# jonathan-laurent/AlphaZero.jl

Hardware: AMD Instinct MI355X
Metric: self-play MCTS sims/sec (Connect-Four, 4096 parallel games per GPU) (higher is better)
Workload: dtype f32

## Files before the change

### alphazero.jl_amd/csrc/net.hip

```cpp
#include "engine.h"

#define AZ_NET_DECL(sfx)                                                                                                     \
  int net_set_kernel_attrs_##sfx(az_engine* e);                                                                                       \
  int net_launch_##sfx(az_engine* e, hipStream_t st, bool from_planes, float* hfeat, const GEnv* envs, const int* eslots,    \
                       const int* n_ptr, int n_max, const float* X, const float* Amask, float* Pout, float* Vout, float* Pinv, \
                       int pstride);                                                                                         \
  int net_wave_##sfx(az_engine* e, int g, bool split, int nmax);                                                             \
  int net_geometry_##sfx(int which, uint16_t* out, int64_t cap, int* rows, int* products);
AZ_NET_DECL(c4)
AZ_NET_DECL(ttt)
AZ_NET_DECL(mancala)
AZ_NET_DECL(go9)

int net_set_kernel_attrs(az_engine* e) {
  switch (e->cfg.game) {
    case AZ_GAME_CONNECT_FOUR: return net_set_kernel_attrs_c4(e);
    case AZ_GAME_TICTACTOE: return net_set_kernel_attrs_ttt(e);
    case AZ_GAME_MANCALA: return net_set_kernel_attrs_mancala(e);
    case AZ_GAME_GO9_PLANES: return net_set_kernel_attrs_go9(e);
  }
  return fail(AZ_ERR_BAD_ARG, "unknown game id %d", e->cfg.game);
}
int net_launch(az_engine* e, hipStream_t st, bool from_planes, float* hfeat, const GEnv* envs, const int* eslots, const int* n_ptr,
               int n_max, const float* X, const float* Amask, float* Pout, float* Vout, float* Pinv, int pstride) {
  switch (e->cfg.game) {
    case AZ_GAME_CONNECT_FOUR: return net_launch_c4(e, st, from_planes, hfeat, envs, eslots, n_ptr, n_max, X, Amask, Pout, Vout, Pinv, pstride);
    case AZ_GAME_TICTACTOE: return net_launch_ttt(e, st, from_planes, hfeat, envs, eslots, n_ptr, n_max, X, Amask, Pout, Vout, Pinv, pstride);
    case AZ_GAME_MANCALA: return net_launch_mancala(e, st, from_planes, hfeat, envs, eslots, n_ptr, n_max, X, Amask, Pout, Vout, Pinv, pstride);
    case AZ_GAME_GO9_PLANES: return net_launch_go9(e, st, from_planes, hfeat, envs, eslots, n_ptr, n_max, X, Amask, Pout, Vout, Pinv, pstride);
  }
  return fail(AZ_ERR_BAD_ARG, "unknown game id %d", e->cfg.game);
}
int net_wave(az_engine* e, int g, bool split, int nmax) {
  switch (e->cfg.game) {
    case AZ_GAME_CONNECT_FOUR: return net_wave_c4(e, g, split, nmax);
    case AZ_GAME_TICTACTOE: return net_wave_ttt(e, g, split, nmax);
    case AZ_GAME_MANCALA: return net_wave_mancala(e, g, split, nmax);
    case AZ_GAME_GO9_PLANES: return net_wave_go9(e, g, split, nmax);
  }
  return fail(AZ_ERR_BAD_ARG, "unknown game id %d", e->cfg.game);
}

extern "C" int az_debug_tower_geometry(int32_t game, int32_t which, uint16_t* out, int64_t cap, int32_t* rows, int32_t* products) {
  if (!out || !rows || !products || which < 0 || which > 3) return fail(AZ_ERR_BAD_ARG, "bad argument");
  switch (game) {
    case AZ_GAME_CONNECT_FOUR: return net_geometry_c4(which, out, cap, rows, products);
    case AZ_GAME_TICTACTOE: return net_geometry_ttt(which, out, cap, rows, products);
    case AZ_GAME_MANCALA: return net_geometry_mancala(which, out, cap, rows, products);
    case AZ_GAME_GO9_PLANES: return net_geometry_go9(which, out, cap, rows, products);
  }
  return fail(AZ_ERR_BAD_ARG, "unknown game id %d", game);
}
```

### alphazero.jl_amd/csrc/net_c4.hip

```cpp
#include "net_impl.h"
AZ_NET_GAME_TU(ConnectFour, c4)


template <int F, int NT> static int tower_timeline(az_engine* e, int32_t n, unsigned long long* out, int64_t cap) {
  using T = T16<ConnectFour, F, NT>;
  const int nb = (n + T::TB - 1) / T::TB;
  if (cap < (int64_t)nb * 8) return fail(AZ_ERR_CAPACITY, "need %d words", nb * 8);
  unsigned long long* d = nullptr;
  AZCHK(dalloc(e, &d, (size_t)nb * 8));
  HIPCHK(hipMemsetAsync(d, 0, sizeof(unsigned long long) * nb * 8, e->stream));
  std::vector<GEnv> envs(n, ConnectFour::init());
  HIPCHK(hipMemcpyAsync(e->d_tmp_env, envs.data(), sizeof(GEnv) * n, hipMemcpyHostToDevice, e->stream));
  HIPCHK(hipMemcpyAsync(e->d_ntmp, &n, sizeof(int), hipMemcpyHostToDevice, e->stream));
  Net16Dev nd = e->net16;
  for (int rep = 0; rep < 2; ++rep) {
    nd.dbg = rep ? d : nullptr;
    hipLaunchKernelGGL((k_tower16<ConnectFour, F, false, NT>), dim3(nb), dim3(T::THREADS), T::BYTES, e->stream, nd, e->d_tmp_env, e->d_iota, e->d_ntmp, n, (const float*)nullptr, e->d_hfeat);
  }
  HIPCHK(hipMemcpyAsync(out, d, sizeof(unsigned long long) * nb * 8, hipMemcpyDeviceToHost, e->stream));
  HIPCHK(hipStreamSynchronize(e->stream));
  e->allocs.pop_back();
  (void)hipFree(d);
  return AZ_OK;
}
static int tower_timeline_split(az_engine* e, int32_t n, unsigned long long* out, int64_t cap) {
  using T = T16S<ConnectFour, 128>;
  const int nb = 2 * ((n + T::TB - 1) / T::TB);
  if (nb > e->num_cu) return fail(AZ_ERR_BAD_ARG, "split tower: at most %d boards", e->num_cu / 2 * T::TB);
  if (cap < (int64_t)nb * 8) return fail(AZ_ERR_CAPACITY, "need %d words", nb * 8);
  unsigned long long* d = nullptr;
  AZCHK(dalloc(e, &d, (size_t)nb * 8));
  std::vector<GEnv> envs(n, ConnectFour::init());
  HIPCHK(hipMemcpyAsync(e->d_tmp_env, envs.data(), sizeof(GEnv) * n, hipMemcpyHostToDevice, e->stream));
  HIPCHK(hipMemcpyAsync(e->d_ntmp, &n, sizeof(int), hipMemcpyHostToDevice, e->stream));
  unsigned long long* xa; unsigned long long ep;
  Net16Dev nd = e->net16;
  for (int rep = 0; rep < 2; ++rep) {
    nd.dbg = rep ? d : nullptr;
    AZCHK(xch_slot<ConnectFour>(e, e->d_hfeat, &xa, &ep));
    hipLaunchKernelGGL((k_tower16s<ConnectFour, 128, false>), dim3(nb), dim3(T::THREADS), T::BYTES, e->stream, nd, e->d_tmp_env, e->d_iota, e->d_ntmp, n, (const float*)nullptr, e->d_hfeat,
                       xa, ep, e->v.err, e->d_xflag);
  }
  HIPCHK(hipMemcpyAsync(out, d, sizeof(unsigned long long) * nb * 8, hipMemcpyDeviceToHost, e->stream));
  HIPCHK(hipStreamSynchronize(e->stream));
  e->allocs.pop_back();
  (void)hipFree(d);
  return AZ_OK;
}
template <int F> static int tower_timeline_bf16(az_engine* e, int32_t n, unsigned long long* out, int64_t cap) {
  using T = T16B<ConnectFour, F, 11>;
  const int nb = (n + T::TB - 1) / T::TB;
  if (cap < (int64_t)nb * 8) return fail(AZ_ERR_CAPACITY, "need %d words", nb * 8);
  unsigned long long* d = nullptr;
  AZCHK(dalloc(e, &d, (size_t)nb * 8));
  std::vector<GEnv> envs(n, ConnectFour::init());
  HIPCHK(hipMemcpyAsync(e->d_tmp_env, envs.data(), sizeof(GEnv) * n, hipMemcpyHostToDevice, e->stream));
  HIPCHK(hipMemcpyAsync(e->d_ntmp, &n, sizeof(int), hipMemcpyHostToDevice, e->stream));
  Net16bDev nd = e->net16b;
  for (int rep = 0; rep < 2; ++rep) {
    nd.dbg = rep ? d : nullptr;
    hipLaunchKernelGGL((k_tower16b<ConnectFour, F, false, 11>), dim3(nb), dim3(T::THREADS), T::BYTES, e->stream, nd, e->d_tmp_env, e->d_iota, e->d_ntmp, n, (const float*)nullptr, e->d_hfeat);
  }
  HIPCHK(hipMemcpyAsync(out, d, sizeof(unsigned long long) * nb * 8, hipMemcpyDeviceToHost, e->stream));
  HIPCHK(hipStreamSynchronize(e->stream));
  e->allocs.pop_back();
  (void)hipFree(d);
  return AZ_OK;
}
template <int F> static int heads_timeline(az_engine* e, int32_t n, unsigned long long* out, int64_t cap) {
  using H = H16<ConnectFour, F, true>;
  const int nb = 2 * ((n + 15) / 16);
  if (cap < (int64_t)nb * H::WAVES * 4) return fail(AZ_ERR_CAPACITY, "need %d words", nb * H::WAVES * 4);
  unsigned long long* d = nullptr;
  AZCHK(dalloc(e, &d, (size_t)nb * H::WAVES * 4));
  std::vector<GEnv> envs(n, ConnectFour::init());
  HIPCHK(hipMemcpyAsync(e->d_tmp_env, envs.data(), sizeof(GEnv) * n, hipMemcpyHostToDevice, e->stream));
  HIPCHK(hipMemcpyAsync(e->d_ntmp, &n, sizeof(int), hipMemcpyHostToDevice, e->stream));
  AZCHK(net_launch(e, e->stream, false, e->d_hfeat, e->d_tmp_env, e->d_iota, e->d_ntmp, n, nullptr, nullptr, e->d_P, e->d_V, nullptr, ConnectFour::A));
  NetDev nd = e->net;
  nd.dbg = d;
  hipLaunchKernelGGL((k_heads16<ConnectFour, F, true>), dim3(nb), dim3(H::THREADS), H::BYTES, e->stream, nd, e->d_tmp_env, e->d_iota, e->d_ntmp, n, (const float*)nullptr, e->d_hfeat, e->d_P, e->d_V, (float*)nullptr, ConnectFour::A);
  HIPCHK(hipMemcpyAsync(out, d, sizeof(unsigned long long) * nb * H::WAVES * 4, hipMemcpyDeviceToHost, e->stream));
  HIPCHK(hipStreamSynchronize(e->stream));
  e->allocs.pop_back();
  (void)hipFree(d);
  return AZ_OK;
}
extern "C" int az_debug_exchange_timeout(az_engine* e) {
  ENGINE(e);
  if (e->cfg.oracle != AZ_ORACLE_RESNET || !e->net_loaded || e->cfg.game != AZ_GAME_CONNECT_FOUR || e->cfg.num_filters != 128 || e->cfg.net_bf16) return fail(AZ_ERR_BAD_ARG, "connect-four, ResNet oracle, 128 filters, fp32");
  using T = T16S<ConnectFour, 128>;
  const int n = 2;
  std::vector<GEnv> envs(n, ConnectFour::init());
  HIPCHK(hipMemcpyAsync(e->d_tmp_env, envs.data(), sizeof(GEnv) * n, hipMemcpyHostToDevice, e->stream));
  HIPCHK(hipMemcpyAsync(e->d_ntmp, &n, sizeof(int), hipMemcpyHostToDevice, e->stream));
  unsigned long long* xa; unsigned long long ep;
  AZCHK(xch_slot<ConnectFour>(e, e->d_hfeat, &xa, &ep));
  hipLaunchKernelGGL((k_tower16s<ConnectFour, 128, false>), dim3(2 * n), dim3(T::THREADS), T::BYTES, e->stream, e->net16, e->d_tmp_env, e->d_iota, e->d_ntmp, n, (const float*)nullptr, e->d_hfeat,
                     xa, ep | (1ull << 63), e->v.err, e->d_xflag);
  return check_device_error(e);
}
extern "C" int az_debug_tree_stamps(az_engine* e, unsigned long long* out) {
  ENGINE(e);
  if (!out) {
    unsigned long long* d = nullptr;
    AZCHK(dalloc(e, &d, 16));
    AZCHK(sync_all(e));
    e->v.dbg = d; e->gv[0].dbg = d;
    return AZ_OK;
  }
  if (!e->gv[0].dbg) return fail(AZ_ERR_STATE, "stamps are not enabled");
  AZCHK(sync_all(e));
  HIPCHK(hipMemcpy(out, e->gv[0].dbg, 16 * sizeof(unsigned long long), hipMemcpyDeviceToHost));
  return AZ_OK;
}
extern "C" int az_debug_heads_timeline(az_engine* e, int32_t n, unsigned long long* out, int64_t cap) {
  ENGINE(e);
  if (e->cfg.oracle != AZ_ORACLE_RESNET || !e->net_loaded || n < 1 || n > e->nn_cap || e->cfg.game != AZ_GAME_CONNECT_FOUR || !e->net.hd16_ok) return fail(AZ_ERR_BAD_ARG, "connect-four, ResNet oracle with 32 head filters");
  return e->cfg.num_filters == 128 ? heads_timeline<128>(e, n, out, cap) : heads_timeline<64>(e, n, out, cap);
}
extern "C" int az_debug_tower_timeline(az_engine* e, int32_t n, int32_t nt, unsigned long long* out, int64_t cap) {
  ENGINE(e);
  if (e->cfg.oracle != AZ_ORACLE_RESNET) return fail(AZ_ERR_BAD_ARG, "the tower timeline needs an engine with the ResNet oracle");
  if (!e->net_loaded || n < 1 || n > e->nn_cap) return fail(AZ_ERR_BAD_ARG, "bad n / no net");
  if (e->cfg.game == AZ_GAME_CONNECT_FOUR && e->cfg.net_bf16 && nt == 11) return e->cfg.num_filters == 128 ? tower_timeline_bf16<128>(e, n, out, cap) : tower_timeline_bf16<64>(e, n, out, cap);
  if (e->cfg.game != AZ_GAME_CONNECT_FOUR || e->cfg.net_bf16 || (nt != 11 && nt != 3 && nt != 2)) return fail(AZ_ERR_BAD_ARG, "connect-four; fp32: nt = 11, 3 or 2 (= split tower), bf16: nt = 11");
  if (nt == 2) return e->cfg.num_filters == 128 ? tower_timeline_split(e, n, out, cap) : fail(AZ_ERR_BAD_ARG, "split tower: 128 filters");
  if (e->cfg.num_filters == 64) return nt == 11 ? tower_timeline<64, 11>(e, n, out, cap) : tower_timeline<64, 3>(e, n, out, cap);
  return nt == 11 ? tower_timeline<128, 11>(e, n, out, cap) : tower_timeline<128, 3>(e, n, out, cap);
}
```

### alphazero.jl_amd/csrc/net_impl.h

```cpp
#pragma once
#include "engine.h"

template <class T> static constexpr double geo_frac() { return T::Geo::tab.cost / (9.0 * (T::RPAD / 16)); }
template <class T_, int ID_, bool OK_, int HIST_> struct FormFp32 {
  using T = T_;
  static constexpr int ID = ID_, HIST = HIST_;
  static constexpr bool OK = OK_, BF16 = false, STOP = false;
  static const Net16Dev& net(const az_engine* e) { return e->net16; }
  static constexpr double frac() { return geo_frac<T>(); }
};
template <class Gm, int F, int NT, int ID_, int HIST_> struct Form16 : FormFp32<T16<Gm, F, NT>, ID_, (NT > 0), HIST_> {
  template <bool FP> static constexpr auto K = &k_tower16<Gm, F, FP, NT>;
  static void name(char* s, size_t n, const char* g) { snprintf(s, n, "k_tower16<%s,%d,NT=%d>", g, F, NT); }
};
template <class Gm, int F> struct FormSplit : FormFp32<T16S<Gm, F>, TW_SPLIT, F == 128, 0> {
  template <bool FP> static constexpr auto K = &k_tower16s<Gm, F, FP>;
  static void name(char* s, size_t n, const char* g) { snprintf(s, n, "k_tower16s<%s,%d>", g, F); }
};
template <class Gm, int F, int NT0, int NT1, int ID_> struct FormPaired : FormFp32<T16P<Gm, F, NT0, NT1>, ID_, F == 64, 2> {
  template <bool FP> static constexpr auto K = &k_tower16x2<Gm, F, FP, NT0, NT1>;
  static constexpr bool STOP = true;
  static void name(char* s, size_t n, const char* g) {
    if (NT0 == 11) snprintf(s, n, "k_tower16x2<%s,%d>", g, F);
    else snprintf(s, n, "k_tower16x2<%s,%d,NT=%d>", g, F, NT0 + NT1);
  }
};
template <class Gm, int F> struct FormPairedC : FormFp32<T16P<Gm, F>, TW_P21C, F == 64, 2> {
  template <bool FP> static constexpr auto K = &k_tower16x2c<Gm, F, FP>;
  static constexpr bool STOP = true;
  static void name(char* s, size_t n, const char* g) { snprintf(s, n, "k_tower16x2c<%s,%d>", g, F); }
};
template <class Gm, int F> struct FormMixed : FormFp32<T16P<Gm, F>, TW_MIXED, F == 64, 2> {
  using T7 = T16P<Gm, F, 10, 9>;
  template <bool FP> static constexpr auto K = &k_tower16x2m<Gm, F, FP>;
  static void name(char* s, size_t n, const char* g) { snprintf(s, n, "k_tower16x2m<%s,%d>", g, F); }
};
template <class Gm, int F> struct Form32 {
  struct T { static constexpr int RPAD = TOWER_ROWS, TB = RPAD / Gm::P, THREADS = TowerCfg<F>::THREADS, BYTES = TowerLds<F>::BYTES; };
  static constexpr int ID = TW_32, HIST = 3;
  static constexpr bool OK = true, BF16 = false, STOP = false;
  template <bool FP> static constexpr auto K = &k_tower<Gm, F, FP>;
  static const NetDev& net(const az_engine* e) { return e->net; }
  static constexpr double frac() { return 1.0; }
  static void name(char* s, size_t n, const char* g) { snprintf(s, n, "k_tower<%s,%d>", g, F); }
};
template <class Gm, int F, int NT, int ID_, int HIST_> struct Form16b {
  using T = T16B<Gm, F, NT>;
  static constexpr int ID = ID_, HIST = HIST_;
  static constexpr bool OK = NT != 22 || F == 128, BF16 = true, STOP = false;
  template <bool FP> static constexpr auto K = &k_tower16b<Gm, F, FP, NT>;
  static const Net16bDev& net(const az_engine* e) { return e->net16b; }
  static constexpr double frac() { return geo_frac<T>(); }
  static void name(char* s, size_t n, const char* g) { snprintf(s, n, "k_tower16b<%s,%d,NT=%d>", g, F, NT); }
};
template <class... D> struct FormList {};
template <class Gm, int F> using Forms = FormList<
    FormSplit<Gm, F>, Form16<Gm, F, NTS<Gm>, TW_NTS, 1>, Form16<Gm, F, NTM<Gm>, TW_NTM, 3>, Form16<Gm, F, 11, TW_11, 2>,
    FormPaired<Gm, F, 11, 10, TW_P21>, FormPaired<Gm, F, 10, 9, TW_P19>, FormPairedC<Gm, F>, Form32<Gm, F>,
    Form16b<Gm, F, NTS<Gm>, TW_NTS, 1>, Form16b<Gm, F, 11, TW_11, 2>, Form16b<Gm, F, 22, TW_B22, 3>>;
template <class D, int F> static constexpr TowerFacts facts() {
  if constexpr (!D::OK) return TowerFacts{D::ID, D::BF16};
  else return TowerFacts{D::ID, D::BF16, true, D::STOP, D::T::TB, D::T::RPAD, D::frac(), D::BF16 && F == 64 ? 2 : 1};
}
template <class Gm, int F, class... D> static TowerTable tower_table(FormList<D...>) {
  static constexpr TowerFacts forms[] = {facts<D, F>()...};
  return TowerTable{forms, (int)sizeof...(D), F, Gm::P, Gm::APAD};
}
template <class Gm, int F> static TowerTable tower_table() { return tower_table<Gm, F>(Forms<Gm, F>{}); }

template <class D, bool FP> static int set_form_attr() {
  if constexpr (D::OK) HIPCHK(hipFuncSetAttribute(reinterpret_cast<const void*>(D::template K<FP>), hipFuncAttributeMaxDynamicSharedMemorySize, D::T::BYTES));
  return AZ_OK;
}
template <class Gm, int F, class... D> static int set_kernel_attrs_f(FormList<D...>) {
  int r = AZ_OK;
  (void)(((r = set_form_attr<D, false>()) == AZ_OK && (r = set_form_attr<D, true>()) == AZ_OK) && ...);
  AZCHK(r);
  AZCHK((set_form_attr<FormMixed<Gm, F>, false>()));
  HIPCHK(hipFuncSetAttribute(reinterpret_cast<const void*>(&k_heads16<Gm, F, true>), hipFuncAttributeMaxDynamicSharedMemorySize, H16<Gm, F, true>::BYTES));
  HIPCHK(hipFuncSetAttribute(reinterpret_cast<const void*>(&k_heads16<Gm, F, false>), hipFuncAttributeMaxDynamicSharedMemorySize, H16<Gm, F, false>::BYTES));
  return AZ_OK;
}
template <class T> static int upload_geo(az_engine* e) {
  using G = typename T::Geo;
  if (e->d_geo[T::GEO]) return AZ_OK;
  std::vector<uint16_t> h((size_t)10 * G::RPAD);
  for (int i = 0; i < G::RPAD; ++i) h[i] = G::tab.pos[i];
  for (int i = 0; i < 9 * G::RPAD; ++i) h[G::RPAD + i] = G::tab.nbr[i];
  uint16_t* d = nullptr;
  AZCHK(dalloc(e, &d, h.size(), false));
  HIPCHK(hipMemcpyAsync(d, h.data(), h.size() * sizeof(uint16_t), hipMemcpyHostToDevice, e->stream));
  HIPCHK(hipStreamSynchronize(e->stream));
  e->d_geo[T::GEO] = d;
  return AZ_OK;
}
template <class D> static int upload_form_geo(az_engine* e) {
  if constexpr (D::OK && D::ID != TW_32) AZCHK((upload_geo<typename D::T>(e)));
  return AZ_OK;
}
template <class... D> static int upload_geos(az_engine* e, FormList<D...>) {
  int r = AZ_OK;
  (void)(((r = upload_form_geo<D>(e)) == AZ_OK) && ...);
  return r;
}
template <class G> static int geometry_out(uint16_t* out, int64_t cap, int* rows, int* products) {
  if (cap < (int64_t)10 * G::RPAD) return fail(AZ_ERR_CAPACITY, "need %d words", 10 * G::RPAD);
  for (int i = 0; i < G::RPAD; ++i) out[i] = G::tab.pos[i];
  for (int i = 0; i < 9 * G::RPAD; ++i) out[G::RPAD + i] = G::tab.nbr[i];
  *rows = G::RPAD; *products = G::tab.cost;
  return AZ_OK;
}
static const char* game_name(const az_engine* e);
static int raise_stop_word(az_engine* e, hipStream_t sn) {
  HIPCHK(hipEventRecord(e->fr_ev[3], sn));
  HIPCHK(hipStreamWaitEvent(e->fr_s[3], e->fr_ev[3], 0));
  hipLaunchKernelGGL(k_set_word, dim3(1), dim3(1), 0, e->fr_s[3], e->d_bg_stop, e->bg_seq);
  return AZ_OK;
}
template <class Gm> static constexpr bool SIMPLE_OK = Gm::A <= 16;
template <class Gm> static int simple_set_kernel_attrs() {
  if constexpr (SIMPLE_OK<Gm>) {
    const int most = (int)sn_lds_bytes(sn_row_words(16 * SN_WAVES * SN_TPW));
    HIPCHK(hipFuncSetAttribute(reinterpret_cast<const void*>(&k_simplenet<Gm, false>), hipFuncAttributeMaxDynamicSharedMemorySize, most));
    HIPCHK(hipFuncSetAttribute(reinterpret_cast<const void*>(&k_simplenet<Gm, true>), hipFuncAttributeMaxDynamicSharedMemorySize, most));
  }
  return AZ_OK;
}
template <class Gm, bool FROM_PLANES>
static int launch_simple(az_engine* e, hipStream_t st, const GEnv* envs, const int* eslots, const int* n_ptr, int n_max, const float* X,
                         const float* Amask, float* Pout, float* Vout, float* Pinv, int pstride) {
  if constexpr (!SIMPLE_OK<Gm>) return fail(AZ_ERR_STATE, "no SimpleNet kernel for this geometry");
  else {
    if (n_max <= 0) return AZ_OK;
    snprintf(e->last_tower, sizeof e->last_tower, "k_simplenet<%s>", game_name(e));
    e->tower_hist[3]++;
    LAUNCH_ON(e, st, AZ_K_TOWER, n_max, (k_simplenet<Gm, FROM_PLANES>), (n_max + SN_ROWS - 1) / SN_ROWS, SN_THREADS, sn_lds_bytes(e->snet.rs), e->snet,
              envs, eslots, n_ptr, n_max, X, Amask, Pout, Vout, Pinv, pstride);
    return AZ_OK;
  }
}
template <class Net> static int wave_frame(az_engine* e, int g, bool split, Net net) {
  hipStream_t st = e->gs[g], sn = e->gt[g];
  if (split) { HIPCHK(hipEventRecord(e->ev_tree[g], st)); HIPCHK(hipStreamWaitEvent(sn, e->ev_tree[g], 0)); }
  AZCHK(net(sn));
  if (split) {
    HIPCHK(hipEventRecord(e->ev_net[g], sn));
    if (!e->ph.fr_on) HIPCHK(hipStreamWaitEvent(st, e->ev_net[g], 0));
  }
  return AZ_OK;
}
struct WaveLeaves { int N; const int* nev; const int* eslots; };
static WaveLeaves wave_leaves(const az_engine* e, int g, int nmax) {
  const DView& v = e->gv[g];
  return WaveLeaves{std::max(1, std::min(v.G, nmax)), v.n_eval + e->wave_par[g], v.eval_slots + (size_t)e->wave_par[g] * v.eval_stride};
}
template <class Gm> static int wave_simple(az_engine* e, int g, bool split, int nmax) {
  const DView& v = e->gv[g];
  const WaveLeaves w = wave_leaves(e, g, nmax);
  return wave_frame(e, g, split, [&](hipStream_t sn) -> int {
    AZCHK((launch_simple<Gm, false>(e, sn, v.leaf_env, w.eslots, w.nev, w.N, nullptr, nullptr, v.Pout, v.Vout, nullptr, Gm::APAD)));
    if (e->bg_signal) AZCHK(raise_stop_word(e, sn));
    return AZ_OK;
  });
}

template <class Gm> static int set_kernel_attrs(az_engine* e) {
  if (e->cfg.oracle == AZ_ORACLE_SIMPLENET) return simple_set_kernel_attrs<Gm>();
  AZCHK((set_kernel_attrs_f<Gm, 64>(Forms<Gm, 64>{})));
  AZCHK((set_kernel_attrs_f<Gm, 128>(Forms<Gm, 128>{})));
  memset(e->d_geo, 0, sizeof e->d_geo);
  AZCHK(upload_geos(e, Forms<Gm, 64>{}));
  AZCHK(upload_geos(e, Forms<Gm, 128>{}));
  AZCHK((upload_geo<typename FormMixed<Gm, 64>::T7>(e)));
  AZCHK((upload_geo<T16<Gm, 64, 6>>(e)));
  return AZ_OK;
}

static TowerAsk tower_ask(const az_engine* e, int n) {
  TowerAsk a;
  a.n = n; a.num_cu = e->num_cu; a.ngroups = e->ngroups;
  a.bf16 = e->cfg.net_bf16 != 0; a.num_blocks = e->cfg.num_blocks; a.tower_pick = e->env.tower_pick; a.use_graphs = e->env.use_graphs != 0; a.split_off = e->split_off;
  a.split_streams = split_streams_on_device(e->device);
  return a;
}
template <class Gm> static int xch_slot(az_engine* e, const float* hfeat, unsigned long long** xch, unsigned long long* epoch) {
  using T = T16S<Gm, 128>;
  const size_t words = (size_t)cus(e->num_cu) * T::XCH_WORDS;
  int slot = AZ_MAX_GROUPS;
  for (int g = 0; g < e->ngroups; ++g) if (hfeat == e->g_hfeat[g]) slot = g;
  if (!e->xch[slot]) {
    AZCHK(dalloc(e, &e->xch[slot], words));
    HIPCHK(hipStreamSynchronize(e->stream));
  }
  if (((e->xch_epoch + 1) & 0xFFFFFFull) == 0) {
    AZCHK(sync_all(e));
    for (int k = 0; k <= AZ_MAX_GROUPS; ++k) if (e->xch[k]) HIPCHK(hipMemset(e->xch[k], 0, words * sizeof(unsigned long long)));
    ++e->xch_epoch;
  }
  *xch = e->xch[slot];
  *epoch = ++e->xch_epoch;
  if (e->env.xch_fail_at > 0 && ++e->xch_launches == e->env.xch_fail_at) *epoch |= 1ull << 63;
  return AZ_OK;
}
template <class Gm, int F>
static int launch_heads(az_engine* e, hipStream_t st, const float* hfeat, const GEnv* envs, const int* eslots, const int* n_ptr, int n_max,
                        const float* Amask, float* Pout, float* Vout, float* Pinv, int pstride) {
  const int tiles = (n_max + 15) / 16;
  switch (choose_heads(e->env.heads_pick, e->net.hd16_ok, e->net.hd_ok, n_max, e->ngroups, e->num_cu)) {
    case HD_16_STAGED:
      LAUNCH_ON(e, st, AZ_K_HEADS, n_max, (k_heads16<Gm, F, true>), 2 * tiles, (H16<Gm, F, true>::THREADS), (H16<Gm, F, true>::BYTES), e->net, envs, eslots, n_ptr, n_max, Amask, hfeat, Pout, Vout, Pinv, pstride);
      break;
    case HD_16:
      LAUNCH_ON(e, st, AZ_K_HEADS, n_max, (k_heads16<Gm, F, false>), tiles, (H16<Gm, F, false>::THREADS), (H16<Gm, F, false>::BYTES), e->net, envs, eslots, n_ptr, n_max, Amask, hfeat, Pout, Vout, Pinv, pstride);
      break;
    case HD_MFMA:
      LAUNCH_ON(e, st, AZ_K_HEADS, n_max, (k_heads_mfma<Gm, F>), (n_max + 31) / 32, 64 * (F / 32 + HEADS_NPT<Gm>), 0, e->net, envs, eslots, n_ptr, n_max, Amask, hfeat, Pout, Vout, Pinv, pstride);
      break;
    case HD_VALU:
      LAUNCH_ON(e, st, AZ_K_HEADS, n_max, (k_heads<Gm, F>), (n_max + 3) / 4, 4 * (F + HEADS_LP<Gm>), 0, e->net, envs, eslots, n_ptr, n_max, Amask, hfeat, Pout, Vout, Pinv, pstride);
      break;
  }
  return AZ_OK;
}
struct TowerIn { float* hfeat; const GEnv* envs; const int* eslots; const int* n_ptr; const float* X; int* xerr; int* stop = nullptr; int stop_val = 0; };
static const char* game_name(const az_engine* e) {
  static const char* const gn[] = {"ConnectFour", "TicTacToe", "Mancala", "Go9Planes"};
  return gn[e->cfg.game];
}
template <class D, bool FROM_PLANES> static int launch_form(az_engine* e, hipStream_t st, int n, const TowerIn& in) {
  if constexpr (!D::OK) return fail(AZ_ERR_STATE, "tower form %d does not exist for this network", (int)D::ID);
  else {
    using T = typename D::T;
    D::name(e->last_tower, sizeof e->last_tower, game_name(e));
    e->tower_hist[D::HIST]++;
    e->next_exec = D::frac();
    const int tiles = (n + T::TB - 1) / T::TB;
    if constexpr (D::ID == TW_SPLIT) {
      unsigned long long* xa; unsigned long long ep;
      AZCHK(xch_slot<typename T::Game>(e, in.hfeat, &xa, &ep));
      LAUNCH_ON(e, st, AZ_K_TOWER, n, (D::template K<FROM_PLANES>), T::SPLIT * tiles, T::THREADS, T::BYTES, D::net(e), in.envs, in.eslots, in.n_ptr, n, in.X, in.hfeat,
                xa, ep, in.xerr, e->d_xflag);
    } else if constexpr (D::STOP)
      LAUNCH_ON(e, st, AZ_K_TOWER, n, (D::template K<FROM_PLANES>), tiles, T::THREADS, T::BYTES, D::net(e), in.envs, in.eslots, in.n_ptr, n, in.X, in.hfeat,
                in.stop, in.stop_val, cus(e->num_cu));
    else
      LAUNCH_ON(e, st, AZ_K_TOWER, n, (D::template K<FROM_PLANES>), tiles, T::THREADS, T::BYTES, D::net(e), in.envs, in.eslots, in.n_ptr, n, in.X, in.hfeat);
    return AZ_OK;
  }
}
template <class Gm, int F, bool FROM_PLANES, class... D>
static int launch_tower(FormList<D...>, az_engine* e, hipStream_t st, int form, int n, const TowerIn& in) {
  const bool bf16 = e->cfg.net_bf16 != 0;
  int r = 1;
  (void)((D::ID == form && D::BF16 == bf16 && ((r = launch_form<D, FROM_PLANES>(e, st, n, in)), true)) || ...);
  return r <= 0 ? r : fail(AZ_ERR_STATE, "no tower form %d", form);
}
template <class Gm, int F, bool FROM_PLANES> static int launch_tower(az_engine* e, hipStream_t st, int form, int n, const TowerIn& in) {
  return launch_tower<Gm, F, FROM_PLANES>(Forms<Gm, F>{}, e, st, form, n, in);
}
template <class Gm, int F, bool FROM_PLANES>
static int launch_net_f(az_engine* e, hipStream_t st, float* hfeat, const GEnv* envs, const int* eslots, const int* n_ptr, int n_max, const float* X,
                        const float* Amask, float* Pout, float* Vout, float* Pinv, int pstride) {
  if (n_max <= 0) return AZ_OK;
  AZCHK((launch_tower<Gm, F, FROM_PLANES>(e, st, choose_tower(tower_table<Gm, F>(), tower_ask(e, n_max)), n_max, TowerIn{hfeat, envs, eslots, n_ptr, X, e->v.err})));
  return launch_heads<Gm, F>(e, st, hfeat, envs, eslots, n_ptr, n_max, Amask, Pout, Vout, Pinv, pstride);
}
template <class Gm, bool FROM_PLANES>
static int launch_net(az_engine* e, hipStream_t st, float* hfeat, const GEnv* envs, const int* eslots, const int* n_ptr, int n_max, const float* X,
                      const float* Amask, float* Pout, float* Vout, float* Pinv, int pstride) {
  if (e->cfg.oracle == AZ_ORACLE_SIMPLENET) return launch_simple<Gm, FROM_PLANES>(e, st, envs, eslots, n_ptr, n_max, X, Amask, Pout, Vout, Pinv, pstride);
  if (e->cfg.num_filters == 128) return launch_net_f<Gm, 128, FROM_PLANES>(e, st, hfeat, envs, eslots, n_ptr, n_max, X, Amask, Pout, Vout, Pinv, pstride);
  return launch_net_f<Gm, 64, FROM_PLANES>(e, st, hfeat, envs, eslots, n_ptr, n_max, X, Amask, Pout, Vout, Pinv, pstride);
}


template <class Gm, int F> static int wave_net_f(az_engine* e, int g, bool split, int nmax) {
  const DView& v = e->gv[g];
  const WaveLeaves w = wave_leaves(e, g, nmax);
  const bool fr = e->ph.fr_on && split;
  auto heads = [&](hipStream_t s) -> int {
    return launch_heads<Gm, F>(e, s, e->g_hfeat[g], v.leaf_env, w.eslots, w.nev, w.N, (const float*)nullptr, v.Pout, v.Vout, (float*)nullptr, Gm::APAD);
  };
  AZCHK(wave_frame(e, g, split, [&](hipStream_t sn) -> int {
    TowerAsk ask = tower_ask(e, w.N);
    ask.fr_on = e->ph.fr_on; ask.fr_kbg = e->ph.fr_kbg; ask.tower_mixed = e->env.tower_mixed; ask.bg_signal = e->bg_signal;
    if (v.nleaf_host) ask.seen = ((volatile int*)e->h_nleaf)[g];
    if (v.needy_host) { ask.needy = ((volatile int*)e->h_needy)[g]; ask.needy_on = true; }
    const WaveTower tw = choose_wave_tower(tower_table<Gm, F>(), ask);
    TowerIn in{e->g_hfeat[g], v.leaf_env, w.eslots, w.nev, nullptr, v.xerr};
    if (tw.tower_stops) { in.stop = e->d_bg_stop; in.stop_val = e->bg_seq; }
    if constexpr (FormMixed<Gm, F>::OK) {
      if (tw.mixed) {
        using M = FormMixed<Gm, F>;
        using T8 = typename M::T; using T7 = typename M::T7;
        const int cu = cus(e->num_cu), first = cu * T8::TB;
        M::name(e->last_tower, sizeof e->last_tower, game_name(e));
        e->tower_hist[M::HIST]++;
        e->next_exec = (first * geo_frac<T8>() + (ask.seen - first) * geo_frac<T7>()) / (double)ask.seen;
        LAUNCH_ON(e, sn, AZ_K_TOWER, w.N, (M::template K<false>), cu + (w.N - first + T7::TB - 1) / T7::TB, T8::THREADS, T8::BYTES, M::net(e), in.envs, in.eslots, in.n_ptr, w.N, in.X, in.hfeat, cu, in.stop, in.stop_val);
      }
    }
    if (!tw.mixed) AZCHK((launch_tower<Gm, F, false>(e, sn, tw.form, w.N, in)));
    if (e->bg_signal && !tw.tower_stops) AZCHK(raise_stop_word(e, sn));
    return fr ? heads(sn) : AZ_OK;
  }));
  return fr ? AZ_OK : heads(e->gs[g]);
}
template <class Gm> static int wave_net(az_engine* e, int g, bool split, int nmax) {
  if (e->cfg.oracle == AZ_ORACLE_SIMPLENET) return wave_simple<Gm>(e, g, split, nmax);
  return e->cfg.num_filters == 128 ? wave_net_f<Gm, 128>(e, g, split, nmax) : wave_net_f<Gm, 64>(e, g, split, nmax);
}

#define AZ_NET_GAME_TU(Gm, sfx)                                                                                              \
  int net_set_kernel_attrs_##sfx(az_engine* e) { return set_kernel_attrs<Gm>(e); }                                                      \
  int net_launch_##sfx(az_engine* e, hipStream_t st, bool from_planes, float* hfeat, const GEnv* envs, const int* eslots,    \
                       const int* n_ptr, int n_max, const float* X, const float* Amask, float* Pout, float* Vout, float* Pinv, \
                       int pstride) {                                                                                        \
    return from_planes ? launch_net<Gm, true>(e, st, hfeat, envs, eslots, n_ptr, n_max, X, Amask, Pout, Vout, Pinv, pstride)  \
                       : launch_net<Gm, false>(e, st, hfeat, envs, eslots, n_ptr, n_max, X, Amask, Pout, Vout, Pinv, pstride); \
  }                                                                                                                          \
  int net_wave_##sfx(az_engine* e, int g, bool split, int nmax) { return wave_net<Gm>(e, g, split, nmax); }                  \
  int net_geometry_##sfx(int which, uint16_t* out, int64_t cap, int* rows, int* products) {                                  \
    return which == 0 ? geometry_out<typename T16<Gm, 64, 11>::Geo>(out, cap, rows, products)                                \
         : which == 1 ? geometry_out<typename T16<Gm, 64, NTS<Gm>>::Geo>(out, cap, rows, products)                                 \
         : which == 2 ? geometry_out<typename T16P<Gm, 64>::Geo>(out, cap, rows, products)                                   \
                      : geometry_out<typename T16B<Gm, 128, 22>::Geo>(out, cap, rows, products);                             \
  }
```

### alphazero.jl_amd/csrc/resnet16.h

```cpp
#pragma once
#include <hip/hip_runtime.h>
#include <stdint.h>
#include "../../include/az_numerics.h"
#include "games.h"
#include "resnet.h"


enum GeoSlot {
  GEO_11,
  GEO_NTS,
  GEO_21,
  GEO_6,
  GEO_NTM,
  GEO_19,
  GEO_22,
  GEO_COUNT
};
struct Net16Dev {
  int nblocks;
  const float* stem_w;
  const float* stem_ss;
  const float4* conv_w;
  const float* conv_ss;
  const float4* head_w;
  const float* head_ss;
  const uint16_t* geo[GEO_COUNT];
  unsigned long long* dbg;
};
static constexpr int GEO_NZ = 8;
template <class Gm, int NTILES, int TBOARDS> struct Geo16 {
  static constexpr int P = Gm::P, W = Gm::W, H = Gm::H, RPAD = NTILES * 16, ROWS = TBOARDS * P, NPADR = RPAD - ROWS;
  static_assert(NPADR >= 0, "boards do not fit the tiles");
  struct Tab {
    uint16_t pos[RPAD];
    uint16_t nbr[9 * RPAD];
    uint16_t tapmask[NTILES];
    int cost;
    int la, lb, lg, off;
  };
  static constexpr int lres(int a, int b, int g, int cell) {
    const int bd = cell / P, q = cell % P;
    return (a * (q % W) + b * (q / W) + g * bd) & 7;
  }
  static constexpr int cls(int q) {
    const int x = q % W, y = q / W;
    if (W >= 2 && x == 0) return 1;
    if (W >= 2 && x == W - 1) return 2;
    if (y == 0) return H == 1 ? 0 : 3;
    if (y == H - 1) return 4;
    return 0;
  }
  static constexpr int valid9(int q) {
    int m = 0;
    for (int tap = 0; tap < 9; ++tap) {
      const int x = q % W + (tap % 3 - 1), y = q / W + (tap / 3 - 1);
      if (x >= 0 && x < W && y >= 0 && y < H) m |= 1 << tap;
    }
    return m;
  }
  struct Order { int ord[5]; };
  static constexpr Order order_of(int order_code) {
    Order o{{0, 1, 2, 3, 4}};
    int pool[4] = {1, 2, 3, 4}, n = 4, code = order_code;
    for (int i = 0; i < 4; ++i) {
      const int k = code % n; code /= n;
      o.ord[1 + i] = pool[k];
      for (int j = k; j + 1 < n; ++j) pool[j] = pool[j + 1];
      --n;
    }
    return o;
  }
  static constexpr int cost_of(int order_code, int padpos) {
    const Order o = order_of(order_code);
    int v9[P] = {}, ncls[5] = {};
    for (int q = 0; q < P; ++q) { v9[q] = valid9(q); ncls[cls(q)]++; }
    int cost = 0, r = 0, mask = 0;
    auto put = [&](int m, int count) {
      for (int k = 0; k < count; ++k) {
        mask |= m;
        if (++r % 16 == 0) { for (int t = 0; t < 9; ++t) cost += (mask >> t) & 1; mask = 0; }
      }
    };
    for (int ci = 0; ci < 5; ++ci) {
      for (int b = 0; b < TBOARDS; ++b)
        for (int q = 0; q < P; ++q) if (cls(q) == o.ord[ci]) put(v9[q], 1);
      if (ci == padpos) put(0, NPADR);
    }
    return cost;
  }
  static constexpr int arrange(int order_code, int padpos, int a, int b, int g, bool same_taps, uint16_t (&out)[RPAD]) {
    const Order o = order_of(order_code);
    int v9[P] = {};
    for (int q = 0; q < P; ++q) v9[q] = valid9(q);
    uint16_t cells[RPAD] = {};
    uint8_t res[RPAD] = {};
    int r = 0, off = 0;
    for (int ci = 0; ci < 5; ++ci) {
      int n = 0;
      for (int bd = 0; bd < TBOARDS; ++bd)
        for (int q = 0; q < P; ++q) if (cls(q) == o.ord[ci]) { cells[n] = (uint16_t)(bd * P + q); res[n] = (uint8_t)lres(a, b, g, bd * P + q); ++n; }
      bool used[RPAD] = {};
      for (int i = 0; i < n; ++i) {
        const int want = (r + i) & 7, v = v9[cells[i] % P];
        out[r + i] = 0xfffe;
        for (int j = 0; j < n; ++j)
          if (!used[j] && res[j] == want && (!same_taps || v9[cells[j] % P] == v)) { out[r + i] = cells[j]; used[j] = true; break; }
      }
      for (int i = 0; i < n; ++i) if (out[r + i] == 0xfffe) {
        const int v = v9[cells[i] % P];
        for (int j = 0; j < n; ++j) if (!used[j] && (!same_taps || v9[cells[j] % P] == v)) { out[r + i] = cells[j]; used[j] = true; ++off; break; }
      }
      r += n;
      if (ci == padpos) for (int k = 0; k < NPADR; ++k) out[r++] = 0xffff;
    }
    return off;
  }
  static constexpr int products(const uint16_t (&pos)[RPAD]) {
    int cost = 0;
    for (int t = 0; t < NTILES; ++t) {
      int m = 0;
      for (int i = 0; i < 16; ++i) if (pos[t * 16 + i] != 0xffff) m |= valid9(pos[t * 16 + i] % P);
      for (int tap = 0; tap < 9; ++tap) cost += (m >> tap) & 1;
    }
    return cost;
  }
  static constexpr int mismatch(int order_code, int padpos, int a, int b, int g) {
    const Order o = order_of(order_code);
    int r = 0, off = 0;
    for (int ci = 0; ci < 5; ++ci) {
      int have[8] = {}, n = 0;
      for (int q = 0; q < P; ++q) if (cls(q) == o.ord[ci])
        for (int bd = 0; bd < TBOARDS; ++bd) { have[(a * (q % W) + b * (q / W) + g * bd) & 7]++; ++n; }
      for (int k = 0; k < 8; ++k) {
        const int need = n / 8 + (((k - r) & 7) < n % 8 ? 1 : 0);
        off += have[k] > need ? have[k] - need : 0;
      }
      r += n;
      if (ci == padpos) r += NPADR;
    }
    return off;
  }
  static constexpr Tab build(int order_code, int padpos) {
    Tab t{};
    int ba = 0, bb = 0, bg = 0, boff = RPAD + 1;
    for (int a = 0; a < 8; ++a)
      for (int b = 0; b < 8; ++b)
        for (int g = 0; g < 8; ++g) {
          const int off = mismatch(order_code, padpos, a, b, g);
          if (off < boff) { boff = off; ba = a; bb = b; bg = g; }
        }
    t.la = ba; t.lb = bb; t.lg = bg;
    t.off = arrange(order_code, padpos, ba, bb, bg, false, t.pos);
    if (products(t.pos) > cost_of(order_code, padpos)) t.off = arrange(order_code, padpos, ba, bb, bg, true, t.pos);
    uint16_t row_of[ROWS > 0 ? ROWS : 1] = {};
    for (int i = 0; i < RPAD; ++i) if (t.pos[i] != 0xffff) row_of[t.pos[i]] = (uint16_t)i;
    for (int i = 0; i < NTILES; ++i) t.tapmask[i] = 0;
    for (int i = 0; i < RPAD; ++i) {
      for (int tap = 0; tap < 9; ++tap) {
        const int dx = tap % 3 - 1, dy = tap / 3 - 1;
        int nb = RPAD + ((i + ba * dx + bb * dy + 16) & 7);
        if (t.pos[i] != 0xffff) {
          const int b = t.pos[i] / P, q = t.pos[i] % P, x = q % W + dx, y = q / W + dy;
          if (x >= 0 && x < W && y >= 0 && y < H) { nb = row_of[b * P + y * W + x]; t.tapmask[i / 16] |= (uint16_t)(1u << tap); }
        }
        t.nbr[tap * RPAD + i] = (uint16_t)nb;
      }
    }
    t.cost = 0;
    for (int i = 0; i < NTILES; ++i) for (int tap = 0; tap < 9; ++tap) t.cost += (t.tapmask[i] >> tap) & 1;
    return t;
  }
  static constexpr Tab best() {
    int bo = 0, bp = 4, bc = cost_of(0, 4);
    for (int oc = 0; oc < 24; ++oc)
      for (int pp = 0; pp < 5; ++pp) {
        const int c = cost_of(oc, pp);
        if (c < bc) { bc = c; bo = oc; bp = pp; }
      }
    return build(bo, bp);
  }
  static constexpr Tab tab = best();
};

template <class Gm> constexpr int NTS = Gm::P <= 48 ? 3 : (Gm::P + 15) / 16;
template <class Gm> constexpr int ntm_of() { for (int nt = 4; nt <= 10; ++nt) if ((16 * nt) % Gm::P == 0) return nt; return Gm::P == 42 ? 6 : 0; }
template <class Gm> constexpr int NTM = ntm_of<Gm>();
template <class Gm, int F = 64, int NT = 11> struct T16 {
  static constexpr int NTILE = NT, RPAD = NTILE * 16;
  static constexpr int TB = RPAD / Gm::P;
  static constexpr int ROWS = TB * Gm::P;
  static constexpr int STRIDE = F + 8;
  static constexpr int BUF = (RPAD + GEO_NZ) * STRIDE;
  static constexpr int PLANES = (RPAD + GEO_NZ) * Gm::C;
  static constexpr int TABLE = (10 * RPAD + 1) / 2;
  static constexpr int BYTES = (BUF + PLANES + TABLE) * 4;
  static constexpr int WAVES = F / 16, THREADS = 64 * WAVES;
  static constexpr int CT = F / 16;
  static constexpr int KH = F / 64;
  static constexpr int SQ = F / 16;
  using Game = Gm;
  using Geo = Geo16<Gm, NTILE, TB>;
  static constexpr GeoSlot GEO = NT == 11 ? GEO_11 : NT == NTS<Gm> ? GEO_NTS : NT == NTM<Gm> ? GEO_NTM : GEO_6;
  static_assert(GEO != GEO_6 || NT == 6, "no table slot for this tile count");
  static constexpr int FILT = F;
};
template <class Gm, int F = 64, int NT0_ = 11, int NT1_ = 10> struct T16P {
  static constexpr int NT0 = NT0_, NT1 = NT1_, NTW = NT0 + NT1, RPAD = NTW * 16;
  static constexpr int TB = RPAD / Gm::P;
  static constexpr int ROWS = TB * Gm::P;
  static constexpr int STRIDE = F + 8;
  static constexpr int BUF = (RPAD + GEO_NZ) * STRIDE;
  static constexpr int PLANES = (RPAD + GEO_NZ) * Gm::C;
  static constexpr int TABLE = (10 * RPAD + 1) / 2;
  static constexpr int BYTES = (BUF + PLANES + TABLE) * 4;
  static constexpr int CT = F / 16, WAVES = 2 * CT, THREADS = 64 * WAVES;
  static constexpr int KH = F / 64, SQ = F / 16;
  using Game = Gm;
  using Geo = Geo16<Gm, NTW, TB>;
  static constexpr GeoSlot GEO = NT0 == 11 ? GEO_21 : GEO_19;
  static_assert(NTW == 21 || NTW == 19, "no table slot for this tile count");
  static constexpr int FILT = F;
};

template <int F> __device__ __forceinline__ int posF(int c) {
  const int G = (c >= F / 2 ? 1 : 0) + 2 * (c & 1), w = (c % (F / 2)) >> 1;
  return (w >> 4) * 64 + ((w >> 2) & 3) * 16 + G * 4 + (w & 3);
}

static constexpr int T16_GMAX = 2;

template <class G, int NT, int TILE0, int KH, int NTAP> struct Steps16 {
  static constexpr int MAXS = 9 * KH * ((NT + 1) / 2);
  struct L {
    int n;
    int8_t tap[MAXS], kh[MAXS], t0[MAXS], t1[MAXS];
    int8_t first[MAXS];
    int8_t next_tap[MAXS];
    int8_t ord[MAXS];
    int8_t first_tap;
  };
  static constexpr L make() {
    L l{};
    l.n = 0; l.first_tap = -1;
    int taps[9] = {}, ntaps = 0;
    for (int tap = 0; tap < 9; ++tap) {
      if (NTAP == 1 && tap != 4) continue;
      bool any = false;
      for (int t = 0; t < NT; ++t) any = any || ((G::tab.tapmask[TILE0 + t] >> tap) & 1);
      if (any) taps[ntaps++] = tap;
    }
    for (int ti = 0; ti < ntaps; ++ti) {
      const int tap = taps[ti];
      if (l.first_tap < 0) l.first_tap = (int8_t)tap;
      int act[NT] = {}, na = 0;
      for (int t = 0; t < NT; ++t) if ((G::tab.tapmask[TILE0 + t] >> tap) & 1) act[na++] = t;
      for (int kh = 0; kh < KH; ++kh)
        for (int i = 0; i < na; i += 2) {
          const int k = l.n++;
          l.tap[k] = (int8_t)tap; l.kh[k] = (int8_t)kh; l.t0[k] = (int8_t)act[i]; l.t1[k] = (int8_t)(i + 1 < na ? act[i + 1] : -1);
          l.first[k] = (kh == 0 && i == 0);
          l.next_tap[k] = (int8_t)(ti + 1 < ntaps ? taps[ti + 1] : -1);
          l.ord[k] = (int8_t)ti;
        }
    }
    return l;
  }
  static constexpr L list = make();
};

template <class T>
__device__ __forceinline__ void load_rows16p(const float* __restrict__ buf, int off0, int off1, bool two, int kh, int g, float4 (&a)[T16_GMAX][4]) {
  const float* p0 = buf + off0 + kh * 64 + g * 4;
#pragma unroll
  for (int q = 0; q < 4; ++q) a[0][q] = *(const float4*)(p0 + q * 16);
  if (two) {
    const float* p1 = buf + off1 + kh * 64 + g * 4;
#pragma unroll
    for (int q = 0; q < 4; ++q) a[1][q] = *(const float4*)(p1 + q * 16);
  }
}
template <int T0, int T1, int KHI, int SQ, int NT>
__device__ __forceinline__ void mfma_tiles16(const float4 (&a)[T16_GMAX][4], const float4 (&bfull)[SQ], f32x4v (&acc)[NT]) {
  const float4* b = bfull + KHI * 4;
#pragma unroll
  for (int q = 0; q < 4; ++q) {
    acc[T0] = __builtin_amdgcn_mfma_f32_16x16x4f32(a[0][q].x, b[q].x, acc[T0], 0, 0, 0);
    if constexpr (T1 >= 0) acc[T1] = __builtin_amdgcn_mfma_f32_16x16x4f32(a[1][q].x, b[q].x, acc[T1], 0, 0, 0);
    acc[T0] = __builtin_amdgcn_mfma_f32_16x16x4f32(a[0][q].y, b[q].y, acc[T0], 0, 0, 0);
    if constexpr (T1 >= 0) acc[T1] = __builtin_amdgcn_mfma_f32_16x16x4f32(a[1][q].y, b[q].y, acc[T1], 0, 0, 0);
    acc[T0] = __builtin_amdgcn_mfma_f32_16x16x4f32(a[0][q].z, b[q].z, acc[T0], 0, 0, 0);
    if constexpr (T1 >= 0) acc[T1] = __builtin_amdgcn_mfma_f32_16x16x4f32(a[1][q].z, b[q].z, acc[T1], 0, 0, 0);
    acc[T0] = __builtin_amdgcn_mfma_f32_16x16x4f32(a[0][q].w, b[q].w, acc[T0], 0, 0, 0);
    if constexpr (T1 >= 0) acc[T1] = __builtin_amdgcn_mfma_f32_16x16x4f32(a[1][q].w, b[q].w, acc[T1], 0, 0, 0);
  }
}
template <class T, class SL, int K, int TILE0>
__device__ __forceinline__ void load_idx16p(const uint16_t* __restrict__ nbr, int lrow, int (&idx)[2]) {
  if constexpr (K < SL::list.n) {
    constexpr int tap = SL::list.tap[K], t0 = SL::list.t0[K], t1 = SL::list.t1[K];
    idx[0] = (int)nbr[tap * T::RPAD + (TILE0 + t0) * 16 + lrow] * T::STRIDE;
    if constexpr (t1 >= 0) idx[1] = (int)nbr[tap * T::RPAD + (TILE0 + t1) * 16 + lrow] * T::STRIDE;
  }
}
template <class T, class SL, int NT, int TILE0, int K>
__device__ __forceinline__ void conv16p_steps(const float* __restrict__ buf, const uint16_t* __restrict__ nbr, const float4* __restrict__ wl,
                                              f32x4v (&acc)[NT], int lrow, int g, float4 (&b0)[T::FILT / 16], float4 (&b1)[T::FILT / 16],
                                              float4 (&aA)[T16_GMAX][4], float4 (&aB)[T16_GMAX][4], int (&idx)[2]) {
  constexpr int F = T::FILT;
  if constexpr (K < SL::list.n) {
    constexpr int kh = SL::list.kh[K], t0 = SL::list.t0[K], t1 = SL::list.t1[K], ord = SL::list.ord[K];
    float4 (&cur)[T16_GMAX][4] = (K & 1) ? aB : aA;
    float4 (&nxt)[T16_GMAX][4] = (K & 1) ? aA : aB;
    float4 (&bc)[F / 16] = (ord & 1) ? b1 : b0;
    float4 (&bn)[F / 16] = (ord & 1) ? b0 : b1;
    if constexpr (SL::list.first[K] && SL::list.next_tap[K] >= 0) {
      constexpr int ntap = SL::list.next_tap[K];
#pragma unroll
      for (int q = 0; q < T::SQ; ++q) bn[q] = wl[(size_t)(ntap * T::CT * T::SQ + q) * 64];
    }
    if constexpr (K + 1 < SL::list.n) {
      load_rows16p<T>(buf, idx[0], idx[1], SL::list.t1[K + 1] >= 0, SL::list.kh[K + 1], g, nxt);
      load_idx16p<T, SL, K + 2, TILE0>(nbr, lrow, idx);
    }
    mfma_tiles16<t0, t1, kh, F / 16, NT>(cur, bc, acc);
    __builtin_amdgcn_sched_barrier(0);
    conv16p_steps<T, SL, NT, TILE0, K + 1>(buf, nbr, wl, acc, lrow, g, b0, b1, aA, aB, idx);
  }
}
template <class T, class G, int NT, int TILE0, int NTAP>
__device__ __forceinline__ void conv16p(const float* __restrict__ buf, const uint16_t* __restrict__ nbr, const float4* __restrict__ wl,
                                        f32x4v (&acc)[NT], int lrow, int g) {
  constexpr int F = T::FILT;
  using SL = Steps16<G, NT, TILE0, T::KH, NTAP>;
  if constexpr (SL::list.n > 0) {
    float4 b0[F / 16], b1[F / 16], aA[T16_GMAX][4], aB[T16_GMAX][4];
    int idx[2] = {0, 0};
    constexpr int tap0 = NTAP == 1 ? 0 : SL::list.first_tap;
#pragma unroll
    for (int q = 0; q < F / 16; ++q) b0[q] = wl[(size_t)(tap0 * T::CT * T::SQ + q) * 64];
    load_idx16p<T, SL, 0, TILE0>(nbr, lrow, idx);
    load_rows16p<T>(buf, idx[0], idx[1], SL::list.t1[0] >= 0, SL::list.kh[0], g, aA);
    load_idx16p<T, SL, 1, TILE0>(nbr, lrow, idx);
    __builtin_amdgcn_sched_barrier(0);
    conv16p_steps<T, SL, NT, TILE0, 0>(buf, nbr, wl, acc, lrow, g, b0, b1, aA, aB, idx);
  }
}

template <int F> struct T16Threads { static constexpr int V = 64 * (F / 16); };

struct NoXch {
  static constexpr int STEM_HALVES = 1;
  static constexpr bool EARLY_PUBLISH = false;
};
enum { DERR_EXCHANGE = 6 };
static constexpr unsigned long long XCH_WAIT_TICKS = 5000000ull;
struct PairXch {
  static constexpr int STEM_HALVES = 2;
  unsigned long long* mine;
  const unsigned long long* theirs;
  uint32_t tag0;
  int* err;
  int* hflag;
  int pch;
  static constexpr bool EARLY_PUBLISH = true;
  template <class T, int NT>
  __device__ __forceinline__ void publish(int step, const float (&ov)[NT][4], int tid) const {
    const uint32_t tag = tag0 + (uint32_t)step;
    unsigned long long* m = mine + (size_t)(step & 1) * NT * 4 * T::THREADS + tid;
#pragma unroll
    for (int t = 0; t < NT; ++t)
#pragma unroll
      for (int i = 0; i < 4; ++i)
        __hip_atomic_store(m + (t * 4 + i) * T::THREADS, ((unsigned long long)tag << 32) | __float_as_uint(ov[t][i]), __ATOMIC_RELAXED, __HIP_MEMORY_SCOPE_AGENT);
  }
  template <class T, int NT, int R0>
  __device__ __forceinline__ void collect(int step, float* __restrict__ buf, int g, int lrow, int tid) const {
    constexpr int THREADS = T::THREADS, F = T::FILT;
    const uint32_t tag = tag0 + (uint32_t)step;
    const unsigned long long* th = theirs + (size_t)(step & 1) * NT * 4 * THREADS + tid;
    unsigned long long pv[NT][4];
    int spins = 0;
    unsigned long long t_start = 0;
    for (;;) {
      bool ok = true;
#pragma unroll
      for (int t = 0; t < NT; ++t)
#pragma unroll
        for (int i = 0; i < 4; ++i) {
          pv[t][i] = __hip_atomic_load(th + (t * 4 + i) * THREADS, __ATOMIC_RELAXED, __HIP_MEMORY_SCOPE_AGENT);
          ok = ok && (uint32_t)(pv[t][i] >> 32) == tag;
        }
      if (ok) break;
      if ((++spins & 255) == 0) {
        const unsigned long long now = wall_clock64();
        if (!t_start) t_start = now;
        else if (now - t_start > XCH_WAIT_TICKS) {
          atomicCAS(err, 0, (int)DERR_EXCHANGE);
          if (hflag) __hip_atomic_store(hflag, 1, __ATOMIC_RELAXED, __HIP_MEMORY_SCOPE_SYSTEM);
          break;
        }
      }
    }
    const int ppos = posF<F>(pch);
#pragma unroll
    for (int t = 0; t < NT; ++t)
#pragma unroll
      for (int i = 0; i < 4; ++i) buf[(R0 + t * 16 + g * 4 + i) * T::STRIDE + ppos] = __uint_as_float((uint32_t)pv[t][i]);
    __syncthreads();
  }
};

template <class T, bool FROM_PLANES, int NT, int TILE0, class X = NoXch>
__device__ __forceinline__ void tower16_wave(const Net16Dev& net, float* __restrict__ buf, const float* __restrict__ planes,
                                             const uint16_t* __restrict__ nbr, const uint16_t* __restrict__ pos, int cw,
                                             int lane, int n, int board0, float* __restrict__ hfeat, const X& xch = X{},
                                             int* stop = nullptr, int stop_val = 0) {
  using Gm = typename T::Game;
  using G = typename T::Geo;
  constexpr int F = T::FILT, P = Gm::P, C = Gm::C, TB = T::TB, STRIDE = T::STRIDE, R0 = TILE0 * 16;
  const int lrow = lane & 15, g = lane >> 4;
  unsigned long long* dbg = (net.dbg && threadIdx.x == 0) ? net.dbg + (size_t)blockIdx.x * 8 : nullptr;
#define AZ_STAMP16(i) do { if (dbg) dbg[i] = __builtin_readcyclecounter(); } while (0)
  AZ_STAMP16(0);
  const int ch = cw * 16 + lrow;
  const int opos = posF<F>(ch);

  f32x4v acc[NT];
  float ov[NT][4];
  float xres[NT][4];
#pragma unroll
  for (int hh = 0; hh < X::STEM_HALVES; ++hh) {
    constexpr int KK = 9 * C, K2 = (KK + 1) / 2, NS = (2 * K2 + 3) / 4;
    const int cws = X::STEM_HALVES == 1 ? cw : hh * (F / 32) + cw % (F / 32);
    const int chs = cws * 16 + lrow, oposs = posF<F>(chs);
#pragma unroll
    for (int t = 0; t < NT; ++t) acc[t] = f32x4v{0.f, 0.f, 0.f, 0.f};
#pragma unroll
    for (int s = 0; s < NS; ++s) {
      const float bw = net.stem_w[(size_t)(cws * NS + s) * 64 + lane];
      const int p = 4 * s + g;
      const int k = (p & 1) * K2 + (p >> 1);
      const bool kin = k < KK && p < 2 * K2;
      const int tap = kin ? k / C : 4, c = kin ? k % C : 0;
#pragma unroll
      for (int tile = 0; tile < NT; ++tile) {
        const int row = kin ? (int)nbr[tap * T::RPAD + R0 + tile * 16 + lrow] : T::RPAD;
        const float a = planes[row * C + c];
        acc[tile] = __builtin_amdgcn_mfma_f32_16x16x4f32(a, bw, acc[tile], 0, 0, 0);
      }
    }
    const float sc = net.stem_ss[chs], sh = net.stem_ss[F + chs];
#pragma unroll
    for (int tile = 0; tile < NT; ++tile)
#pragma unroll
      for (int i = 0; i < 4; ++i) {
        const float v = az_fmaf(acc[tile][i], sc, sh);
        const float r = v > 0.0f ? v : 0.0f;
        buf[(R0 + tile * 16 + g * 4 + i) * STRIDE + oposs] = r;
        if (cws == cw) xres[tile][i] = r;
      }
  }
  __syncthreads();
  AZ_STAMP16(1);

  const size_t LAYER_W = (size_t)9 * T::CT * T::SQ * 64;
  for (int layer = 0; layer < 2 * net.nblocks; ++layer) {
#pragma unroll
    for (int t = 0; t < NT; ++t) acc[t] = f32x4v{0.f, 0.f, 0.f, 0.f};
    int lrow_l = lrow;
    asm volatile("" : "+v"(lrow_l));
    conv16p<T, G, NT, TILE0, 9>(buf, nbr, net.conv_w + (size_t)layer * LAYER_W + (size_t)cw * T::SQ * 64 + lane, acc, lrow_l, g);
    const float sc = net.conv_ss[(size_t)layer * 2 * F + ch], sh = net.conv_ss[(size_t)layer * 2 * F + F + ch];
    if (layer == 2) AZ_STAMP16(4);
    if constexpr (X::EARLY_PUBLISH) {
#pragma unroll
      for (int tile = 0; tile < NT; ++tile)
#pragma unroll
        for (int i = 0; i < 4; ++i) {
          float v = az_fmaf(acc[tile][i], sc, sh);
          if (layer & 1) v = v + xres[tile][i];
          ov[tile][i] = v > 0.0f ? v : 0.0f;
          if (layer & 1) xres[tile][i] = ov[tile][i];
        }
      xch.template publish<T, NT>(layer, ov, threadIdx.x);
      __builtin_amdgcn_s_setprio(2);
      __syncthreads();
      if (layer == 2) AZ_STAMP16(5);
#pragma unroll
      for (int tile = 0; tile < NT; ++tile)
#pragma unroll
        for (int i = 0; i < 4; ++i) buf[(R0 + tile * 16 + g * 4 + i) * STRIDE + opos] = ov[tile][i];
      xch.template collect<T, NT, R0>(layer, buf, g, lrow, threadIdx.x);
    } else {
    __builtin_amdgcn_s_setprio(2);
    __syncthreads();
    if (layer == 2) AZ_STAMP16(5);
    if (!(layer & 1)) {
#pragma unroll
      for (int tile = 0; tile < NT; ++tile)
#pragma unroll
        for (int i = 0; i < 4; ++i) {
          const int a = (R0 + tile * 16 + g * 4 + i) * STRIDE + opos;
          const float v = az_fmaf(acc[tile][i], sc, sh);
          buf[a] = v > 0.0f ? v : 0.0f;
        }
    } else {
#pragma unroll
      for (int tile = 0; tile < NT; ++tile)
#pragma unroll
        for (int i = 0; i < 4; ++i) {
          const int a = (R0 + tile * 16 + g * 4 + i) * STRIDE + opos;
          float v = az_fmaf(acc[tile][i], sc, sh);
          v = v + xres[tile][i];
          xres[tile][i] = v > 0.0f ? v : 0.0f;
          buf[a] = xres[tile][i];
        }
    }
    __syncthreads();
    }
    __builtin_amdgcn_s_setprio(0);
    if (layer == 1 || layer == 2) AZ_STAMP16(5 + layer);
  }
  AZ_STAMP16(2);
  if (stop && threadIdx.x == 0) __hip_atomic_store(stop, stop_val, __ATOMIC_RELAXED, __HIP_MEMORY_SCOPE_AGENT);
#pragma unroll
  for (int t = 0; t < NT; ++t) acc[t] = f32x4v{0.f, 0.f, 0.f, 0.f};
  conv16p<T, G, NT, TILE0, 1>(buf, nbr, net.head_w + (size_t)cw * T::SQ * 64 + lane, acc, lrow, g);
  {
    const float sc = net.head_ss[ch], sh = net.head_ss[F + ch];
    const int nvalid = ((n - board0) < TB ? (n - board0) : TB) * P;
#pragma unroll
    for (int tile = 0; tile < NT; ++tile)
#pragma unroll
      for (int i = 0; i < 4; ++i) {
        const int ps = pos[R0 + tile * 16 + g * 4 + i];
        const float v = az_fmaf(acc[tile][i], sc, sh);
        if (ps < nvalid) hfeat[((size_t)board0 * P + ps) * F + ch] = v > 0.0f ? v : 0.0f;
      }
  }
  AZ_STAMP16(3);
#undef AZ_STAMP16
}

template <class T, bool FROM_PLANES>
__device__ __forceinline__ void tower16_fill(float* __restrict__ buf, float* __restrict__ planes, uint16_t* __restrict__ nbr,
                                             uint16_t* __restrict__ pos, const uint16_t* __restrict__ geo, const GEnv* __restrict__ leaf_env,
                                             const int* __restrict__ eval_slots, const float* __restrict__ X, int n, int board0, int tid) {
  using Gm = typename T::Game;
  constexpr int P = Gm::P, C = Gm::C;
  for (int i = tid; i < T::PLANES; i += T::THREADS) {
    const int row = i / C, c = i % C;
    float val = 0.0f;
    if (row < T::RPAD) {
      const int ps = geo[row];
      if (ps != 0xffff && board0 + ps / P < n) {
        const int b = ps / P, q = ps % P;
        if (FROM_PLANES) val = X[((size_t)(board0 + b) * C + c) * P + q];
        else val = Gm::plane(leaf_env[eval_slots[board0 + b]], q, c);
      }
    }
    planes[i] = val;
  }
  for (int i = tid; i < GEO_NZ * T::STRIDE; i += T::THREADS) buf[T::RPAD * T::STRIDE + i] = 0.0f;
  for (int i = tid; i < T::RPAD; i += T::THREADS) pos[i] = geo[i];
  for (int i = tid; i < 9 * T::RPAD; i += T::THREADS) nbr[i] = geo[T::RPAD + i];
}

template <class Gm, int F, bool FROM_PLANES, int NT = 11>
__global__ void __launch_bounds__(T16Threads<F>::V, 2)
k_tower16(Net16Dev net, const GEnv* __restrict__ leaf_env, const int* __restrict__ eval_slots,
          const int* __restrict__ n_eval_ptr, int n_fixed, const float* __restrict__ X, float* __restrict__ hfeat) {
  using T = T16<Gm, F, NT>;
  extern __shared__ __attribute__((aligned(16))) float lds[];
  float* buf = lds;
  float* planes = lds + T::BUF;
  uint16_t* nbr = (uint16_t*)(planes + T::PLANES);
  uint16_t* pos = nbr + 9 * T::RPAD;
  const int n = FROM_PLANES ? n_fixed : *n_eval_ptr;
  const int board0 = blockIdx.x * T::TB;
  if (board0 >= n) return;
  tower16_fill<T, FROM_PLANES>(buf, planes, nbr, pos, net.geo[T::GEO], leaf_env, eval_slots, X, n, board0, threadIdx.x);
  __syncthreads();
  tower16_wave<T, FROM_PLANES, NT, 0>(net, buf, planes, nbr, pos, threadIdx.x >> 6, threadIdx.x & 63, n, board0, hfeat);
}

template <class T, bool FROM_PLANES>
__device__ __forceinline__ void tower16x2_body(const Net16Dev& net, const GEnv* __restrict__ leaf_env, const int* __restrict__ eval_slots, int n,
                                               const float* __restrict__ X, float* __restrict__ hfeat, int board0, const uint16_t* __restrict__ geo,
                                               int* stop = nullptr, int stop_val = 0) {
  extern __shared__ __attribute__((aligned(16))) float lds[];
  float* buf = lds;
  float* planes = lds + T::BUF;
  uint16_t* nbr = (uint16_t*)(planes + T::PLANES);
  uint16_t* pos = nbr + 9 * T::RPAD;
  tower16_fill<T, FROM_PLANES>(buf, planes, nbr, pos, geo, leaf_env, eval_slots, X, n, board0, threadIdx.x);
  __syncthreads();
  const int wave = threadIdx.x >> 6, lane = threadIdx.x & 63;
  if (wave < T::CT) tower16_wave<T, FROM_PLANES, T::NT0, 0>(net, buf, planes, nbr, pos, wave, lane, n, board0, hfeat, NoXch{}, stop, stop_val);
  else tower16_wave<T, FROM_PLANES, T::NT1, T::NT0>(net, buf, planes, nbr, pos, wave - T::CT, lane, n, board0, hfeat);
}
__device__ __forceinline__ int* paired_last_round(int* stop, int wg, int nwg, int num_cu) {
  return stop && wg >= (nwg - 1) / num_cu * num_cu ? stop : nullptr;
}
template <class Gm, int F, bool FROM_PLANES, int NT0 = 11, int NT1 = 10>
__global__ void __launch_bounds__(2 * T16Threads<F>::V, 1)
k_tower16x2(Net16Dev net, const GEnv* __restrict__ leaf_env, const int* __restrict__ eval_slots,
            const int* __restrict__ n_eval_ptr, int n_fixed, const float* __restrict__ X, float* __restrict__ hfeat,
            int* stop, int stop_val, int num_cu) {
  using T = T16P<Gm, F, NT0, NT1>;
  const int n = FROM_PLANES ? n_fixed : *n_eval_ptr;
  const int board0 = blockIdx.x * T::TB;
  if (board0 >= n) return;
  tower16x2_body<T, FROM_PLANES>(net, leaf_env, eval_slots, n, X, hfeat, board0, net.geo[T::GEO], paired_last_round(stop, blockIdx.x, (n + T::TB - 1) / T::TB, num_cu), stop_val);
}
template <class Gm, int F, bool FROM_PLANES>
__global__ void __launch_bounds__(2 * T16Threads<F>::V, 1) __attribute__((amdgpu_num_vgpr(88)))
k_tower16x2c(Net16Dev net, const GEnv* __restrict__ leaf_env, const int* __restrict__ eval_slots,
             const int* __restrict__ n_eval_ptr, int n_fixed, const float* __restrict__ X, float* __restrict__ hfeat,
             int* stop, int stop_val, int num_cu) {
  using T = T16P<Gm, F, 11, 10>;
  const int n = FROM_PLANES ? n_fixed : *n_eval_ptr;
  const int board0 = blockIdx.x * T::TB;
  if (board0 >= n) return;
  tower16x2_body<T, FROM_PLANES>(net, leaf_env, eval_slots, n, X, hfeat, board0, net.geo[T::GEO], paired_last_round(stop, blockIdx.x, (n + T::TB - 1) / T::TB, num_cu), stop_val);
}
template <class Gm, int F, bool FROM_PLANES>
__global__ void __launch_bounds__(2 * T16Threads<F>::V, 1)
k_tower16x2m(Net16Dev net, const GEnv* __restrict__ leaf_env, const int* __restrict__ eval_slots,
             const int* __restrict__ n_eval_ptr, int n_fixed, const float* __restrict__ X, float* __restrict__ hfeat, int first,
             int* stop, int stop_val) {
  using T8 = T16P<Gm, F, 11, 10>;
  using T7 = T16P<Gm, F, 10, 9>;
  const int n = FROM_PLANES ? n_fixed : *n_eval_ptr;
  if ((int)blockIdx.x < first) {
    const int board0 = blockIdx.x * T8::TB;
    if (board0 >= n) return;
    tower16x2_body<T8, FROM_PLANES>(net, leaf_env, eval_slots, n, X, hfeat, board0, net.geo[T8::GEO],
                                    n <= first * T8::TB ? stop : nullptr, stop_val);
  } else {
    const int board0 = first * T8::TB + ((int)blockIdx.x - first) * T7::TB;
    if (board0 >= n) return;
    tower16x2_body<T7, FROM_PLANES>(net, leaf_env, eval_slots, n, X, hfeat, board0, net.geo[T7::GEO], stop, stop_val);
  }
}

template <class Gm, int F> struct T16S : T16<Gm, F, NTS<Gm>> {
  static constexpr int SPLIT = 2, TPW = NTS<Gm>, CWL = F / 16 / SPLIT;
  static constexpr int WAVES = CWL, THREADS = 64 * WAVES;
  static constexpr int XCH_WORDS = 2 * TPW * 4 * THREADS;
};
template <class Gm, int F, bool FROM_PLANES>
__global__ void __launch_bounds__((T16S<Gm, F>::THREADS), 1)
k_tower16s(Net16Dev net, const GEnv* __restrict__ leaf_env, const int* __restrict__ eval_slots,
           const int* __restrict__ n_eval_ptr, int n_fixed, const float* __restrict__ X, float* __restrict__ hfeat,
           unsigned long long* __restrict__ xch, unsigned long long epoch, int* __restrict__ err, int* __restrict__ hflag) {
  using T = T16S<Gm, F>;
  extern __shared__ __attribute__((aligned(16))) float lds[];
  float* buf = lds;
  float* planes = lds + T::BUF;
  uint16_t* nbr = (uint16_t*)(planes + T::PLANES);
  uint16_t* pos = nbr + 9 * T::RPAD;
  const int n = FROM_PLANES ? n_fixed : *n_eval_ptr;
  const int pair = blockIdx.x >> 1, half = blockIdx.x & 1;
  const int board0 = pair * T::TB;
  if (board0 >= n) return;
  if (__hip_atomic_load(err, __ATOMIC_RELAXED, __HIP_MEMORY_SCOPE_AGENT) == (int)DERR_EXCHANGE) return;
  if ((epoch >> 63) && blockIdx.x == 1) return;
  tower16_fill<T, FROM_PLANES>(buf, planes, nbr, pos, net.geo[T::GEO], leaf_env, eval_slots, X, n, board0, threadIdx.x);
  __syncthreads();
  const int wave = threadIdx.x >> 6, lane = threadIdx.x & 63;
  const int cwl = wave;
  PairXch x;
  x.mine = xch + (size_t)blockIdx.x * T::XCH_WORDS;
  x.theirs = xch + (size_t)(blockIdx.x ^ 1) * T::XCH_WORDS;
  x.tag0 = (uint32_t)(epoch << 8);
  x.err = err;
  x.hflag = hflag;
  x.pch = ((half ^ 1) * T::CWL + cwl) * 16 + (lane & 15);
  tower16_wave<T, FROM_PLANES, T::TPW, 0, PairXch>(net, buf, planes, nbr, pos, half * T::CWL + cwl, lane, n, board0, hfeat, x);
}

struct TrFinal {
  int mode;
  long long R; float momentum;
  const float* bias; float *mean, *invstd, *run_mean, *run_var;
  float *dgamma, *dbeta, *mf;
  float* out0;
  int* counter;
};
__device__ __forceinline__ void part_store(double* p, double v) { __hip_atomic_store(p, v, __ATOMIC_RELAXED, __HIP_MEMORY_SCOPE_AGENT); }
__device__ __forceinline__ double part_load(const double* p) { return __hip_atomic_load(p, __ATOMIC_RELAXED, __HIP_MEMORY_SCOPE_AGENT); }
__device__ __forceinline__ void tr_finish(const double* __restrict__ part, int C, const TrFinal& f, double* __restrict__ scratch) {
  if (!f.counter) return;
  __shared__ int s_last;
  __builtin_amdgcn_s_waitcnt(0);
  __syncthreads();
  if (threadIdx.x == 0) s_last = __hip_atomic_fetch_add(f.counter, 1, __ATOMIC_RELEASE, __HIP_MEMORY_SCOPE_AGENT) == (int)(gridDim.x * gridDim.y) - 1;
  __syncthreads();
  if (!s_last) return;
  __builtin_amdgcn_fence(__ATOMIC_ACQUIRE, "agent");
  const int nparts = (int)gridDim.x, T = (int)blockDim.x, t = (int)threadIdx.x, npair = 2 * C;
  double* fin = scratch + T;
  if (npair <= T) {
    const int nsub = T / npair, pair = t % npair, sub = t / npair, w = pair / C, c = pair % C;
    double acc = 0.0;
    if (sub < nsub) for (int k = sub; k < nparts; k += nsub) acc += part_load(part + ((size_t)k * 2 + w) * C + c);
    scratch[t] = acc;
    __syncthreads();
    if (sub == 0) { double v = scratch[pair]; for (int q = 1; q < nsub; ++q) v += scratch[pair + q * npair]; fin[pair] = v; }
  } else {
    for (int pair = t; pair < npair; pair += T) {
      const int w = pair / C, c = pair % C;
      double acc = 0.0;
      for (int k = 0; k < nparts; ++k) acc += part_load(part + ((size_t)k * 2 + w) * C + c);
      fin[pair] = acc;
    }
  }
  __syncthreads();
  for (int c = t; c < C; c += T) {
    const double s0 = fin[c], s1 = fin[C + c];
    if (f.mode == 1) {
      const double m = s0 / (double)f.R;
      double var = s1 / (double)f.R - m * m;
      if (var < 0.0) var = 0.0;
      f.mean[c] = (float)m;
      f.invstd[c] = (float)(1.0 / __builtin_sqrt(var + 1e-5));
      const float b = f.bias ? f.bias[c] : 0.0f;
      f.run_mean[c] = (1.0f - f.momentum) * f.run_mean[c] + f.momentum * ((float)m + b);
      f.run_var[c] = (1.0f - f.momentum) * f.run_var[c] + f.momentum * (float)(var * ((double)f.R / (double)(f.R - 1)));
    } else if (f.mode == 2) { f.dbeta[c] = (float)s0; f.dgamma[c] = (float)s1; f.mf[c] = (float)(s0 / (double)f.R); f.mf[C + c] = (float)(s1 / (double)f.R); }
    else if (f.mode == 3) f.out0[c] = (float)s0;
  }
  if (t == 0) __hip_atomic_store(f.counter, 0, __ATOMIC_RELAXED, __HIP_MEMORY_SCOPE_AGENT);
}
struct BnIn { const float *g, *mean, *invstd, *gamma, *beta, *res; float* a_out; };

template <class Gm, int F, bool STATS, bool STAMP = false, int NT_ = 11>
__global__ void __launch_bounds__(T16Threads<F>::V, 2)
k_conv16_layer(const float* __restrict__ in, const float4* __restrict__ wfrag, float* __restrict__ out, int nboards, const uint16_t* __restrict__ geo,
               double* __restrict__ part, const float* __restrict__ addend, long long* __restrict__ stamps, BnIn bn = BnIn{}, TrFinal fin = TrFinal{}) {
  long long ts[4] = {0, 0, 0, 0};
  if constexpr (STAMP) ts[0] = wall_clock64();
  using T = T16<Gm, F, NT_>;
  using G = typename T::Geo;
  constexpr int P = Gm::P, STRIDE = T::STRIDE, NT = NT_;
  extern __shared__ __attribute__((aligned(16))) float lds[];
  float* buf = lds;
  uint16_t* nbr = (uint16_t*)(lds + T::BUF + T::PLANES);
  uint16_t* pos = nbr + 9 * T::RPAD;
  const int board0 = blockIdx.x * T::TB;
  if (board0 >= nboards) return;
  const int nb = (nboards - board0) < T::TB ? (nboards - board0) : T::TB;
  const int nvalid = nb * P;
  const int tid = threadIdx.x, lane = tid & 63, wave = tid >> 6;
  const float4* in4 = (const float4*)((bn.g ? bn.g : in) + (size_t)board0 * P * F);
  const float4* res4 = bn.res ? (const float4*)(bn.res + (size_t)board0 * P * F) : nullptr;
  float4* aout4 = bn.g ? (float4*)(bn.a_out + (size_t)board0 * P * F) : nullptr;
  for (int idx = tid; idx < (T::RPAD + GEO_NZ) * (F / 4); idx += T::THREADS) {
    const int row = idx / (F / 4), c4 = idx % (F / 4);
    const int ps = row < T::RPAD ? (int)geo[row] : 0xffff;
    float4 v = ps < nvalid ? in4[(size_t)ps * (F / 4) + c4] : make_float4(0.f, 0.f, 0.f, 0.f);
    if (bn.g && ps < nvalid) {
      const float4 mu = ((const float4*)bn.mean)[c4], is = ((const float4*)bn.invstd)[c4], ga = ((const float4*)bn.gamma)[c4], be = ((const float4*)bn.beta)[c4];
      float4 y;
      y.x = ga.x * ((v.x - mu.x) * is.x) + be.x; y.y = ga.y * ((v.y - mu.y) * is.y) + be.y;
      y.z = ga.z * ((v.z - mu.z) * is.z) + be.z; y.w = ga.w * ((v.w - mu.w) * is.w) + be.w;
      if (res4) { const float4 r = res4[(size_t)ps * (F / 4) + c4]; y.x += r.x; y.y += r.y; y.z += r.z; y.w += r.w; }
      v = make_float4(y.x > 0.0f ? y.x : 0.0f, y.y > 0.0f ? y.y : 0.0f, y.z > 0.0f ? y.z : 0.0f, y.w > 0.0f ? y.w : 0.0f);
      aout4[(size_t)ps * (F / 4) + c4] = v;
    }
    float* dst = buf + row * STRIDE;
    dst[posF<F>(c4 * 4 + 0)] = v.x; dst[posF<F>(c4 * 4 + 1)] = v.y; dst[posF<F>(c4 * 4 + 2)] = v.z; dst[posF<F>(c4 * 4 + 3)] = v.w;
  }
  for (int i = tid; i < T::RPAD; i += T::THREADS) pos[i] = geo[i];
  for (int i = tid; i < 9 * T::RPAD; i += T::THREADS) nbr[i] = geo[T::RPAD + i];
  const int lrow = lane & 15, g = lane >> 4;
  __syncthreads();
  if constexpr (STAMP) ts[1] = wall_clock64();
  f32x4v acc[NT];
#pragma unroll
  for (int t = 0; t < NT; ++t) acc[t] = f32x4v{0.f, 0.f, 0.f, 0.f};
  conv16p<T, G, NT, 0, 9>(buf, nbr, wfrag + (size_t)wave * T::SQ * 64 + lane, acc, lrow, g);
  if constexpr (STAMP) { ts[2] = wall_clock64(); __syncthreads(); }
  const int ch = wave * 16 + lrow;
  float* o = out + (size_t)board0 * P * F;
  double s0 = 0.0, s1 = 0.0;
#pragma unroll
  for (int tile = 0; tile < NT; ++tile)
#pragma unroll
    for (int i = 0; i < 4; ++i) {
      const int ps = pos[tile * 16 + g * 4 + i];
      if (ps < nvalid) {
        o[(size_t)ps * F + ch] = addend ? acc[tile][i] + (addend + (size_t)board0 * P * F)[(size_t)ps * F + ch] : acc[tile][i];
        if constexpr (STATS) { const double v = (double)acc[tile][i]; s0 += v; s1 += v * v; }
      }
    }
  if constexpr (STATS) {
    s0 += __shfl_xor(s0, 16); s1 += __shfl_xor(s1, 16);
    s0 += __shfl_xor(s0, 32); s1 += __shfl_xor(s1, 32);
    if (g == 0) { part_store(part + ((size_t)blockIdx.x * 2) * F + ch, s0); part_store(part + ((size_t)blockIdx.x * 2 + 1) * F + ch, s1); }
    __syncthreads();
    tr_finish(part, F, fin, (double*)lds);
  }
  if constexpr (STAMP) {
    __builtin_amdgcn_s_waitcnt(0);
    ts[3] = wall_clock64();
    if (tid == 0) for (int i = 0; i < 4; ++i) stamps[(size_t)blockIdx.x * 4 + i] = ts[i];
  }
}

template <int F, int CS_ = 1, int RPC_ = 128> struct WG16 {
  static constexpr int TPW = F == 128 ? 3 : 9;
  static constexpr int TG = 9 / TPW;
  static constexpr int CS = CS_;
  static constexpr int FA = F / CS;
  static constexpr int CT = F / 16, WAVES = FA / 16, THREADS = 64 * WAVES;
  static constexpr int RP = RPC_;
  static constexpr int STRIDE_A = FA + 16, STRIDE = F + 16;
  static constexpr int RLS = RP + 8;
  static constexpr int BYTES = ((RP + 1) * STRIDE_A + RP * STRIDE + TPW * RLS) * 4;
  static constexpr int WGS_PER_CU = (RP <= 64 && CS > 1) ? 2 : 1;
  __host__ __device__ static constexpr int tap(int y, int k) {
    constexpr int sel[3][3] = {{0, 8, 4}, {2, 1, 3}, {6, 7, 5}};
    return TPW == 3 ? sel[y][k] : k;
  }
};
template <class Gm, int F, int STAMP = 0, int CS = 1, int RPC = 128>
__global__ void __launch_bounds__((WG16<F, CS, RPC>::THREADS), (WG16<F, CS, RPC>::WGS_PER_CU))
k_wgrad16(const float* __restrict__ a, const float* __restrict__ dg, float* __restrict__ part, int nboards, int nsplits, long long* __restrict__ stamps) {
  long long ts[8] = {0, 0, 0, 0, 0, 0, 0, 0};
  if constexpr (STAMP) ts[0] = wall_clock64();
  using G = WG16<F, CS, RPC>;
  constexpr int P = Gm::P, W = Gm::W, H = Gm::H, STRIDE = G::STRIDE, STRIDE_A = G::STRIDE_A, FA = G::FA, RP = G::RP, CT = G::CT, TPW = G::TPW, RLS = G::RLS;
  constexpr int NBC = RP / P < 1 ? 1 : RP / P;
  static_assert(RP >= P, "a chunk holds at least one board");
  extern __shared__ __attribute__((aligned(16))) float lds[];
  float* As = lds;
  float* Ds = lds + (RP + 1) * STRIDE_A;
  uint32_t* rl = (uint32_t*)(Ds + RP * STRIDE);
  const int tid = threadIdx.x, lane = tid & 63, wave = tid >> 6, lrow = lane & 15, g = lane >> 4;
  const int tgroup = blockIdx.y % G::TG, half = blockIdx.y / G::TG;
  const int bq = nboards / nsplits, br = nboards % nsplits;
  const int b_begin = blockIdx.x * bq + ((int)blockIdx.x < br ? (int)blockIdx.x : br);
  const int b_end = b_begin + bq + ((int)blockIdx.x < br ? 1 : 0);
  constexpr int NPA = RP * (FA / 4) / G::THREADS, NPD = RP * (F / 4) / G::THREADS;
  static_assert(RP * (FA / 4) % G::THREADS == 0 && RP * (F / 4) % G::THREADS == 0, "chunk must divide over the threads");
  float4 pa[NPA], pd[NPD];
  auto prefetch = [&](int b0) {
    const int nbp = (b_end - b0) < NBC ? (b_end - b0) : NBC;
    const int nv = nbp > 0 ? nbp * P : 0;
    const float4* a4 = (const float4*)(a + (size_t)b0 * P * F + half * FA);
    const float4* d4 = (const float4*)(dg + (size_t)b0 * P * F);
#pragma unroll
    for (int q = 0; q < NPA; ++q) {
      const int idx = tid + q * G::THREADS, row = idx / (FA / 4), c4 = idx % (FA / 4);
      pa[q] = row < nv ? a4[(size_t)row * (F / 4) + c4] : make_float4(0.f, 0.f, 0.f, 0.f);
    }
#pragma unroll
    for (int q = 0; q < NPD; ++q) {
      const int idx = tid + q * G::THREADS, row = idx / (F / 4), c4 = idx % (F / 4);
      pd[q] = row < nv ? d4[(size_t)row * (F / 4) + c4] : make_float4(0.f, 0.f, 0.f, 0.f);
    }
  };
  prefetch(b_begin);
  for (int i = tid; i < TPW * RLS; i += G::THREADS) rl[i] = ((uint32_t)RP << 16) | (uint32_t)(RP - 1);
  for (int i = tid; i < STRIDE_A; i += G::THREADS) As[RP * STRIDE_A + i] = 0.0f;
  __syncthreads();
  int cnt[TPW];
#pragma unroll
  for (int k = 0; k < TPW; ++k) {
    const int tap = G::tap(tgroup, k), dy = tap / 3 - 1, dx = tap % 3 - 1;
    cnt[k] = (W - (dx != 0)) * (H - (dy != 0));
  }
  if (tid < TPW * NBC) {
    const int k = tid / NBC, b = tid % NBC;
    const int tap = G::tap(tgroup, k), dy = tap / 3 - 1, dx = tap % 3 - 1;
    int n = b * (W - (dx != 0)) * (H - (dy != 0));
    for (int q = 0; q < P; ++q) {
      const int x = q % W, y = q / W;
      if ((y + dy >= 0) && (y + dy < H) && (x + dx >= 0) && (x + dx < W)) {
        const int r = b * P + q;
        rl[k * RLS + n++] = ((uint32_t)(r + dy * W + dx) << 16) | (uint32_t)r;
      }
    }
  }
  f32x4v acc[TPW][CT];
#pragma unroll
  for (int k = 0; k < TPW; ++k)
#pragma unroll
    for (int j = 0; j < CT; ++j) acc[k][j] = f32x4v{0.f, 0.f, 0.f, 0.f};
  if constexpr (STAMP) ts[1] = wall_clock64();
  for (int b0 = b_begin; b0 < b_end; b0 += NBC) {
    const int nb = (b_end - b0) < NBC ? (b_end - b0) : NBC;
    long long tb = 0;
    if constexpr (STAMP) tb = wall_clock64();
    __syncthreads();
    long long tb1 = 0;
    if constexpr (STAMP) tb1 = wall_clock64();
#pragma unroll
    for (int q = 0; q < NPA; ++q) {
      const int idx = tid + q * G::THREADS, row = idx / (FA / 4), c4 = idx % (FA / 4);
      *(float4*)(As + row * STRIDE_A + c4 * 4) = pa[q];
    }
#pragma unroll
    for (int q = 0; q < NPD; ++q) {
      const int idx = tid + q * G::THREADS, row = idx / (F / 4), c4 = idx % (F / 4);
      *(float4*)(Ds + row * STRIDE + c4 * 4) = pd[q];
    }
    __syncthreads();
    long long tb2 = 0;
    if constexpr (STAMP) tb2 = wall_clock64();
    if (b0 + NBC < b_end) prefetch(b0 + NBC);
    if constexpr (STAMP) { const long long tn = wall_clock64(); if (b0 == b_begin) ts[2] = tn; else { ts[3] += tn - tb; ts[6] += tb1 - tb; ts[7] += tb2 - tb1; } }
#pragma unroll
    for (int k = 0; k < TPW; ++k) {
      const int nsteps = (nb * cnt[k] + 3) >> 2;
      const uint32_t* list = rl + k * RLS + g;
      float bv0[CT], bv1[CT], av0, av1;
      auto load_step = [&](uint32_t e, float (&bv)[CT], float& av) {
        if constexpr (STAMP == 2) {
#pragma unroll
          for (int j = 0; j < CT; ++j) bv[j] = __uint_as_float(e + j);
          av = __uint_as_float(e);
          return;
        }
        const float* dp = Ds + (e & 0xffffu) * STRIDE + lrow;
#pragma unroll
        for (int j = 0; j < CT; ++j) bv[j] = dp[j * 16];
        av = As[(e >> 16) * STRIDE_A + wave * 16 + lrow];
      };
      auto mfma_step = [&](const float (&bv)[CT], float av) {
#pragma unroll
        for (int j = 0; j < CT; ++j) {
          if constexpr (STAMP == 3) acc[k][j][0] += av * bv[j];
          else acc[k][j] = __builtin_amdgcn_mfma_f32_16x16x4f32(av, bv[j], acc[k][j], 0, 0, 0);
        }
      };
      auto interleave = [&]() {
#pragma unroll
        for (int j = 0; j < CT; ++j) {
          __builtin_amdgcn_sched_group_barrier(0x008, 1, 0);
          __builtin_amdgcn_sched_group_barrier(0x002, 3, 0);
          __builtin_amdgcn_sched_group_barrier(0x100, 2, 0);
        }
      };
      uint32_t e0 = list[0], e1 = list[4];
      load_step(e0, bv0, av0);
      for (int s0 = 0; s0 + 2 <= nsteps; s0 += 2) {
        __builtin_amdgcn_sched_barrier(0);
        e0 = list[4 * (s0 + 2)];
        load_step(e1, bv1, av1);
        mfma_step(bv0, av0);
        interleave();
        __builtin_amdgcn_sched_barrier(0);
        e1 = list[4 * (s0 + 3)];
        load_step(e0, bv0, av0);
        mfma_step(bv1, av1);
        interleave();
      }
      __builtin_amdgcn_sched_barrier(0);
      if (nsteps & 1) mfma_step(bv0, av0);
      __builtin_amdgcn_sched_barrier(0);
    }
  }
  if constexpr (STAMP) ts[4] = wall_clock64();
  float* o = part + (size_t)blockIdx.x * 9 * F * F;
#pragma unroll
  for (int k = 0; k < TPW; ++k) {
    const int tap = G::tap(tgroup, k);
#pragma unroll
    for (int j = 0; j < CT; ++j)
#pragma unroll
      for (int i = 0; i < 4; ++i)
        o[((size_t)tap * F + (half * FA + wave * 16 + g * 4 + i)) * F + j * 16 + lrow] = acc[k][j][i];
  }
  if constexpr (STAMP) {
    __builtin_amdgcn_s_waitcnt(0);
    ts[5] = wall_clock64();
    if (tid == 0) for (int i = 0; i < 8; ++i) stamps[((size_t)blockIdx.y * gridDim.x + blockIdx.x) * 8 + i] = ts[i];
  }
}
static __global__ void __launch_bounds__(256) k_wgrad_reduce(const float* __restrict__ part, int nsplit, long long n, float* __restrict__ out) {
  __builtin_amdgcn_s_setprio(3);
  const long long i = ((long long)blockIdx.x * blockDim.x + threadIdx.x) * 2;
  if (i >= n) return;
  float2 s[8];
#pragma unroll
  for (int u = 0; u < 8; ++u) s[u] = make_float2(0.f, 0.f);
  int k = 0;
  for (; k + 8 <= nsplit; k += 8)
#pragma unroll
    for (int u = 0; u < 8; ++u) {
      const float2 v = *(const float2*)(part + (size_t)(k + u) * n + i);
      s[u].x += v.x; s[u].y += v.y;
    }
  for (; k < nsplit; ++k) {
    const float2 v = *(const float2*)(part + (size_t)k * n + i);
    s[0].x += v.x; s[0].y += v.y;
  }
  float2 r;
  r.x = ((s[0].x + s[1].x) + (s[2].x + s[3].x)) + ((s[4].x + s[5].x) + (s[6].x + s[7].x));
  r.y = ((s[0].y + s[1].y) + (s[2].y + s[3].y)) + ((s[4].y + s[5].y) + (s[6].y + s[7].y));
  *(float2*)(out + i) = r;
}
```

### alphazero.jl_amd/csrc/resnet16b.h

```cpp
#pragma once
#include <hip/hip_runtime.h>
#include <stdint.h>
#include "resnet16.h"

typedef __bf16 bf16x8v __attribute__((ext_vector_type(8)));

struct Net16bDev {
  int nblocks;
  const float* stem_w;
  const float* stem_ss;
  const bf16x8v* conv_w;
  const float* conv_ss;
  const bf16x8v* head_w;
  const float* head_ss;
  const uint16_t* geo[GEO_COUNT];
  unsigned long long* dbg;
};

template <class Gm, int F = 128, int NT = 11> struct T16B {
  static constexpr int NTILE = NT, RPAD = NTILE * 16;
  static constexpr int TB = RPAD / Gm::P, ROWS = TB * Gm::P;
  static constexpr int SH = F == 128 ? F + 16 : F + 8;
  static constexpr int BUFH = (RPAD + GEO_NZ) * SH;
  static constexpr int PLANES = (RPAD + GEO_NZ) * Gm::C;
  static constexpr int TABLE = (10 * RPAD + 1) / 2;
  static constexpr int BYTES = BUFH * 2 + (PLANES + TABLE) * 4;
  static constexpr int WAVES = F / 16, THREADS = 64 * WAVES, CT = F / 16, KS = F / 32;
  using Game = Gm;
  using Geo = Geo16<Gm, NTILE, TB>;
  static constexpr GeoSlot GEO = NT == 11 ? GEO_11 : NT == 22 ? GEO_22 : GEO_NTS;
  static_assert(GEO != GEO_NTS || NT == NTS<Gm>, "no table slot for this tile count");
  static constexpr int FILT = F;
  static_assert(BUFH * 2 % 16 == 0 && (SH * 2) % 16 == 0, "rows must stay 16-byte aligned");
};

__device__ __forceinline__ uint16_t f32_to_bf16_bits(float x) { return __builtin_bit_cast(uint16_t, (__bf16)x); }
__device__ __forceinline__ float bf16_bits_to_f32(uint16_t h) { return __builtin_bit_cast(float, (uint32_t)h << 16); }

struct EpiSel { uint32_t s0, s1; bool odd; };
__device__ __forceinline__ EpiSel epi_sel(int lrow) {
  const bool odd = lrow & 1;
  return EpiSel{odd ? 0x01000504u : 0x05040100u, odd ? 0x03020706u : 0x07060302u, odd};
}
template <class T>
__device__ __forceinline__ void store_bf16x4(uint16_t* __restrict__ dst, const EpiSel& es, const float (&v)[4], uint32_t (&packed)[2]) {
  typedef __bf16 bf16x2v __attribute__((ext_vector_type(2)));
  typedef float f32x2v __attribute__((ext_vector_type(2)));
  packed[0] = __builtin_bit_cast(uint32_t, __builtin_convertvector(f32x2v{v[0], v[1]}, bf16x2v));
  packed[1] = __builtin_bit_cast(uint32_t, __builtin_convertvector(f32x2v{v[2], v[3]}, bf16x2v));
  const uint32_t mine = es.odd ? packed[1] : packed[0], send = es.odd ? packed[0] : packed[1];
  const uint32_t recv = (uint32_t)__builtin_amdgcn_update_dpp(0, (int)send, 0xB1, 0xF, 0xF, false);
  *(uint32_t*)dst = __builtin_amdgcn_perm(recv, mine, es.s0);
  *(uint32_t*)(dst + T::SH) = __builtin_amdgcn_perm(recv, mine, es.s1);
}
template <class T> __device__ __forceinline__ uint16_t* epi_dst(uint16_t* __restrict__ buf, int row0, int ch, bool odd) {
  return buf + (row0 + (odd ? 2 : 0)) * T::SH + (ch & ~1);
}

template <class T>
__device__ __forceinline__ void load_rows16b(const uint16_t* __restrict__ buf, int off0, int off1, bool two, int g, bf16x8v (&a)[2][T::KS]) {
  const uint16_t* p0 = buf + off0 + g * 8;
#pragma unroll
  for (int ks = 0; ks < T::KS; ++ks) a[0][ks] = *(const bf16x8v*)(p0 + ks * 32);
  if (two) {
    const uint16_t* p1 = buf + off1 + g * 8;
#pragma unroll
    for (int ks = 0; ks < T::KS; ++ks) a[1][ks] = *(const bf16x8v*)(p1 + ks * 32);
  }
}
template <class T, class SL, int K, int TILE0>
__device__ __forceinline__ void load_idx16b(const uint16_t* __restrict__ nbr, int lrow, int (&idx)[2]) {
  if constexpr (K < SL::list.n) {
    constexpr int tap = SL::list.tap[K], t0 = SL::list.t0[K], t1 = SL::list.t1[K];
    idx[0] = (int)nbr[tap * T::RPAD + (TILE0 + t0) * 16 + lrow] * T::SH;
    if constexpr (t1 >= 0) idx[1] = (int)nbr[tap * T::RPAD + (TILE0 + t1) * 16 + lrow] * T::SH;
  }
}
template <class T>
__device__ __forceinline__ void load_w16b(const bf16x8v* __restrict__ wl, int tap, bf16x8v (&b)[2][T::KS]) {
#pragma unroll
  for (int ct = 0; ct < 2; ++ct)
#pragma unroll
    for (int ks = 0; ks < T::KS; ++ks) b[ct][ks] = wl[(size_t)((tap * T::CT + ct) * T::KS + ks) * 64];
}
template <class T, class SL, int NT, int TILE0, int NTAP, int K>
__device__ __forceinline__ void conv16b_steps(const uint16_t* __restrict__ buf, const uint16_t* __restrict__ nbr, const bf16x8v* __restrict__ wl,
                                              f32x4v (&acc)[NT][2], int lrow, int g, bf16x8v (&b0)[2][T::KS], bf16x8v (&b1)[2][T::KS],
                                              bf16x8v (&aA)[2][T::KS], bf16x8v (&aB)[2][T::KS], int (&idx)[2]) {
  if constexpr (K < SL::list.n) {
    constexpr int t0 = SL::list.t0[K], t1 = SL::list.t1[K], ord = SL::list.ord[K];
    bf16x8v (&cur)[2][T::KS] = (K & 1) ? aB : aA;
    bf16x8v (&nxt)[2][T::KS] = (K & 1) ? aA : aB;
    bf16x8v (&bc)[2][T::KS] = (ord & 1) ? b1 : b0;
    bf16x8v (&bn)[2][T::KS] = (ord & 1) ? b0 : b1;
    if constexpr (SL::list.first[K] && SL::list.next_tap[K] >= 0) load_w16b<T>(wl, NTAP == 1 ? 0 : SL::list.next_tap[K], bn);
    if constexpr (K + 1 < SL::list.n) {
      load_rows16b<T>(buf, idx[0], idx[1], SL::list.t1[K + 1] >= 0, g, nxt);
      load_idx16b<T, SL, K + 2, TILE0>(nbr, lrow, idx);
    }
#pragma unroll
    for (int ks = 0; ks < T::KS; ++ks) {
      acc[t0][0] = __builtin_amdgcn_mfma_f32_16x16x32_bf16(cur[0][ks], bc[0][ks], acc[t0][0], 0, 0, 0);
      acc[t0][1] = __builtin_amdgcn_mfma_f32_16x16x32_bf16(cur[0][ks], bc[1][ks], acc[t0][1], 0, 0, 0);
      if constexpr (t1 >= 0) {
        acc[t1][0] = __builtin_amdgcn_mfma_f32_16x16x32_bf16(cur[1][ks], bc[0][ks], acc[t1][0], 0, 0, 0);
        acc[t1][1] = __builtin_amdgcn_mfma_f32_16x16x32_bf16(cur[1][ks], bc[1][ks], acc[t1][1], 0, 0, 0);
      }
    }
    __builtin_amdgcn_sched_barrier(0);
    conv16b_steps<T, SL, NT, TILE0, NTAP, K + 1>(buf, nbr, wl, acc, lrow, g, b0, b1, aA, aB, idx);
  }
}
template <class T, class G, int NT, int TILE0, int NTAP>
__device__ __forceinline__ void conv16b(const uint16_t* __restrict__ buf, const uint16_t* __restrict__ nbr, const bf16x8v* __restrict__ wl,
                                        f32x4v (&acc)[NT][2], int lrow, int g) {
  using SL = Steps16<G, NT, TILE0, 1, NTAP>;
  if constexpr (SL::list.n > 0) {
    bf16x8v b0[2][T::KS], b1[2][T::KS], aA[2][T::KS], aB[2][T::KS];
    int idx[2] = {0, 0};
    load_w16b<T>(wl, NTAP == 1 ? 0 : SL::list.first_tap, b0);
    load_idx16b<T, SL, 0, TILE0>(nbr, lrow, idx);
    load_rows16b<T>(buf, idx[0], idx[1], SL::list.t1[0] >= 0, g, aA);
    load_idx16b<T, SL, 1, TILE0>(nbr, lrow, idx);
    __builtin_amdgcn_sched_barrier(0);
    conv16b_steps<T, SL, NT, TILE0, NTAP, 0>(buf, nbr, wl, acc, lrow, g, b0, b1, aA, aB, idx);
  }
}

template <class T, int NT, int TILE0>
__device__ __forceinline__ void tower16b_wave(const Net16bDev& net, uint16_t* __restrict__ buf, const float* __restrict__ planes,
                                              const uint16_t* __restrict__ nbr, const uint16_t* __restrict__ pos, int cg, int lane,
                                              int n, int board0, float* __restrict__ hfeat) {
  using Gm = typename T::Game;
  using G = typename T::Geo;
  constexpr int F = T::FILT, P = Gm::P, C = Gm::C, TB = T::TB, R0 = TILE0 * 16;
  const int lrow = lane & 15, g = lane >> 4;
  const int ch0 = cg * 32 + lrow;
  unsigned long long* dbg = (net.dbg && threadIdx.x == 0) ? net.dbg + (size_t)blockIdx.x * 8 : nullptr;
#define AZ_STAMP16B(i) do { if (dbg) dbg[i] = __builtin_readcyclecounter(); } while (0)
  AZ_STAMP16B(0);
  f32x4v acc[NT][2];
  const EpiSel es = epi_sel(lrow);
  uint32_t xres[NT][2][2];
  {
    constexpr int KK = 9 * C, K2 = (KK + 1) / 2, NS = (2 * K2 + 3) / 4;
#pragma unroll
    for (int t = 0; t < NT; ++t) { acc[t][0] = f32x4v{0.f, 0.f, 0.f, 0.f}; acc[t][1] = f32x4v{0.f, 0.f, 0.f, 0.f}; }
#pragma unroll
    for (int s = 0; s < NS; ++s) {
      const float bw0 = net.stem_w[(size_t)((cg * 2) * NS + s) * 64 + lane], bw1 = net.stem_w[(size_t)((cg * 2 + 1) * NS + s) * 64 + lane];
      const int p = 4 * s + g;
      const int k = (p & 1) * K2 + (p >> 1);
      const bool kin = k < KK && p < 2 * K2;
      const int tap = kin ? k / C : 4, c = kin ? k % C : 0;
#pragma unroll
      for (int tile = 0; tile < NT; ++tile) {
        const int row = kin ? (int)nbr[tap * T::RPAD + R0 + tile * 16 + lrow] : T::RPAD;
        const float a = planes[row * C + c];
        acc[tile][0] = __builtin_amdgcn_mfma_f32_16x16x4f32(a, bw0, acc[tile][0], 0, 0, 0);
        acc[tile][1] = __builtin_amdgcn_mfma_f32_16x16x4f32(a, bw1, acc[tile][1], 0, 0, 0);
      }
    }
#pragma unroll
    for (int ct = 0; ct < 2; ++ct) {
      const float sc = net.stem_ss[ch0 + 16 * ct], sh = net.stem_ss[F + ch0 + 16 * ct];
#pragma unroll
      for (int tile = 0; tile < NT; ++tile) {
        float v[4];
#pragma unroll
        for (int i = 0; i < 4; ++i) { const float y = az_fmaf(acc[tile][ct][i], sc, sh); v[i] = y > 0.0f ? y : 0.0f; }
        store_bf16x4<T>(epi_dst<T>(buf, R0 + tile * 16 + g * 4, ch0 + 16 * ct, es.odd), es, v, xres[tile][ct]);
      }
    }
  }
  __syncthreads();
  AZ_STAMP16B(1);

  const size_t LAYER_W = (size_t)9 * T::CT * T::KS * 64;
  for (int layer = 0; layer < 2 * net.nblocks; ++layer) {
#pragma unroll
    for (int t = 0; t < NT; ++t) { acc[t][0] = f32x4v{0.f, 0.f, 0.f, 0.f}; acc[t][1] = f32x4v{0.f, 0.f, 0.f, 0.f}; }
    int lrow_l = lrow;
    asm volatile("" : "+v"(lrow_l));
    conv16b<T, G, NT, TILE0, 9>(buf, nbr, net.conv_w + (size_t)layer * LAYER_W + (size_t)(cg * 2) * T::KS * 64 + lane, acc, lrow_l, g);
    if (layer == 2) AZ_STAMP16B(4);
    __syncthreads();
    if (layer == 2) AZ_STAMP16B(5);
    if (layer & 1) {
#pragma unroll
      for (int ct = 0; ct < 2; ++ct) {
        const float sc = net.conv_ss[(size_t)layer * 2 * F + ch0 + 16 * ct], sh = net.conv_ss[(size_t)layer * 2 * F + F + ch0 + 16 * ct];
#pragma unroll
        for (int tile = 0; tile < NT; ++tile) {
          float v[4];
#pragma unroll
          for (int i = 0; i < 4; ++i) {
            const uint32_t pr = xres[tile][ct][i >> 1];
            const float y = az_fmaf(acc[tile][ct][i], sc, sh) + __builtin_bit_cast(float, (i & 1) ? (pr & 0xffff0000u) : (pr << 16));
            v[i] = y > 0.0f ? y : 0.0f;
          }
          store_bf16x4<T>(epi_dst<T>(buf, R0 + tile * 16 + g * 4, ch0 + 16 * ct, es.odd), es, v, xres[tile][ct]);
        }
      }
    } else {
#pragma unroll
      for (int ct = 0; ct < 2; ++ct) {
        const float sc = net.conv_ss[(size_t)layer * 2 * F + ch0 + 16 * ct], sh = net.conv_ss[(size_t)layer * 2 * F + F + ch0 + 16 * ct];
#pragma unroll
        for (int tile = 0; tile < NT; ++tile) {
          float v[4];
#pragma unroll
          for (int i = 0; i < 4; ++i) { const float y = az_fmaf(acc[tile][ct][i], sc, sh); v[i] = y > 0.0f ? y : 0.0f; }
          uint32_t pk[2];
          store_bf16x4<T>(epi_dst<T>(buf, R0 + tile * 16 + g * 4, ch0 + 16 * ct, es.odd), es, v, pk);
        }
      }
    }
    __syncthreads();
    if (layer == 1 || layer == 2) AZ_STAMP16B(5 + layer);
  }
  AZ_STAMP16B(2);
#pragma unroll
  for (int t = 0; t < NT; ++t) { acc[t][0] = f32x4v{0.f, 0.f, 0.f, 0.f}; acc[t][1] = f32x4v{0.f, 0.f, 0.f, 0.f}; }
  conv16b<T, G, NT, TILE0, 1>(buf, nbr, net.head_w + (size_t)(cg * 2) * T::KS * 64 + lane, acc, lrow, g);
  {
    const int nvalid = ((n - board0) < TB ? (n - board0) : TB) * P;
#pragma unroll
    for (int ct = 0; ct < 2; ++ct) {
      const float sc = net.head_ss[ch0 + 16 * ct], sh = net.head_ss[F + ch0 + 16 * ct];
#pragma unroll
      for (int tile = 0; tile < NT; ++tile)
#pragma unroll
        for (int i = 0; i < 4; ++i) {
          const int ps = pos[R0 + tile * 16 + g * 4 + i];
          const float v = az_fmaf(acc[tile][ct][i], sc, sh);
          if (ps < nvalid) hfeat[((size_t)board0 * P + ps) * F + ch0 + 16 * ct] = v > 0.0f ? v : 0.0f;
        }
    }
  }
  AZ_STAMP16B(3);
#undef AZ_STAMP16B
}

template <class Gm, int F, bool FROM_PLANES, int NT = 11>
__global__ void __launch_bounds__(64 * (F / 16), F == 64 ? 2 : 1)
k_tower16b(Net16bDev net, const GEnv* __restrict__ leaf_env, const int* __restrict__ eval_slots,
           const int* __restrict__ n_eval_ptr, int n_fixed, const float* __restrict__ X, float* __restrict__ hfeat) {
  using T = T16B<Gm, F, NT>;
  constexpr int P = Gm::P, C = Gm::C, TB = T::TB, SH = T::SH, NCG = F / 32, NT0 = (NT + 1) / 2, NT1 = NT / 2;
  extern __shared__ __attribute__((aligned(16))) unsigned char ldsb[];
  uint16_t* buf = (uint16_t*)ldsb;
  float* planes = (float*)(ldsb + (size_t)T::BUFH * 2);
  uint16_t* nbr = (uint16_t*)(planes + T::PLANES);
  uint16_t* pos = nbr + 9 * T::RPAD;
  const int n = FROM_PLANES ? n_fixed : *n_eval_ptr;
  const int board0 = blockIdx.x * TB;
  if (board0 >= n) return;
  const int tid = threadIdx.x, lane = tid & 63, wave = tid >> 6;
  const uint16_t* geo = net.geo[T::GEO];
  for (int i = tid; i < T::PLANES; i += T::THREADS) {
    const int row = i / C, c = i % C;
    float val = 0.0f;
    if (row < T::RPAD) {
      const int ps = geo[row];
      if (ps != 0xffff && board0 + ps / P < n) {
        const int b = ps / P, q = ps % P;
        if (FROM_PLANES) val = X[((size_t)(board0 + b) * C + c) * P + q];
        else val = Gm::plane(leaf_env[eval_slots[board0 + b]], q, c);
      }
    }
    planes[i] = val;
  }
  for (int i = tid; i < GEO_NZ * SH; i += T::THREADS) buf[T::RPAD * SH + i] = 0;
  for (int i = tid; i < T::RPAD; i += T::THREADS) pos[i] = geo[i];
  for (int i = tid; i < 9 * T::RPAD; i += T::THREADS) nbr[i] = geo[T::RPAD + i];
  __syncthreads();
  if (wave < NCG) tower16b_wave<T, NT0, 0>(net, buf, planes, nbr, pos, wave, lane, n, board0, hfeat);
  else tower16b_wave<T, NT1, NT0>(net, buf, planes, nbr, pos, wave - NCG, lane, n, board0, hfeat);
}
```

Before: 8.984 million.

## Balance paired-tower tile sets by tap cost and warm-start conv weight fragments

The paired tower kernel used to split the row tiles contiguously, tiles 0..NT0-1 to one wave group and the rest to the other. It now assigns tiles to the two groups with a compile-time subset-sum partition that balances the total number of active taps (MFMA products). It also carries the first weight fragments of the next convolution across layers (warm start), so each layer does not begin with a cold weight load. The aim is to remove load imbalance between the two wave groups and the weight-fetch latency at layer boundaries. In exchange, tiles are no longer contiguous, which adds per-tile row-offset tables and more register pressure.

```diff
diff --git a/alphazero.jl_amd/csrc/net.hip b/alphazero.jl_amd/csrc/net.hip
--- a/alphazero.jl_amd/csrc/net.hip
+++ b/alphazero.jl_amd/csrc/net.hip
@@ -6,7 +6,8 @@
                        const int* n_ptr, int n_max, const float* X, const float* Amask, float* Pout, float* Vout, float* Pinv, \
                        int pstride);                                                                                         \
   int net_wave_##sfx(az_engine* e, int g, bool split, int nmax);                                                             \
-  int net_geometry_##sfx(int which, uint16_t* out, int64_t cap, int* rows, int* products);
+  int net_geometry_##sfx(int which, uint16_t* out, int64_t cap, int* rows, int* products);                                   \
+  int net_sets_##sfx(int which, int32_t* out, int64_t cap, int* nt0, int* nt1, int* products);
 AZ_NET_DECL(c4)
 AZ_NET_DECL(ttt)
 AZ_NET_DECL(mancala)
@@ -42,7 +43,7 @@
 }
 
 extern "C" int az_debug_tower_geometry(int32_t game, int32_t which, uint16_t* out, int64_t cap, int32_t* rows, int32_t* products) {
-  if (!out || !rows || !products || which < 0 || which > 3) return fail(AZ_ERR_BAD_ARG, "bad argument");
+  if (!out || !rows || !products || which < 0 || which > 4) return fail(AZ_ERR_BAD_ARG, "bad argument");
   switch (game) {
     case AZ_GAME_CONNECT_FOUR: return net_geometry_c4(which, out, cap, rows, products);
     case AZ_GAME_TICTACTOE: return net_geometry_ttt(which, out, cap, rows, products);
@@ -51,3 +52,13 @@
   }
   return fail(AZ_ERR_BAD_ARG, "unknown game id %d", game);
 }
+extern "C" int az_debug_tower_sets(int32_t game, int32_t which, int32_t* out, int64_t cap, int32_t* nt0, int32_t* nt1, int32_t* products) {
+  if (!out || !nt0 || !nt1 || !products || (which != 2 && which != 4)) return fail(AZ_ERR_BAD_ARG, "bad argument");
+  switch (game) {
+    case AZ_GAME_CONNECT_FOUR: return net_sets_c4(which, out, cap, nt0, nt1, products);
+    case AZ_GAME_TICTACTOE: return net_sets_ttt(which, out, cap, nt0, nt1, products);
+    case AZ_GAME_MANCALA: return net_sets_mancala(which, out, cap, nt0, nt1, products);
+    case AZ_GAME_GO9_PLANES: return net_sets_go9(which, out, cap, nt0, nt1, products);
+  }
+  return fail(AZ_ERR_BAD_ARG, "unknown game id %d", game);
+}
diff --git a/alphazero.jl_amd/csrc/net_c4.hip b/alphazero.jl_amd/csrc/net_c4.hip
--- a/alphazero.jl_amd/csrc/net_c4.hip
+++ b/alphazero.jl_amd/csrc/net_c4.hip
@@ -18,6 +18,29 @@
     hipLaunchKernelGGL((k_tower16<ConnectFour, F, false, NT>), dim3(nb), dim3(T::THREADS), T::BYTES, e->stream, nd, e->d_tmp_env, e->d_iota, e->d_ntmp, n, (const float*)nullptr, e->d_hfeat);
   }
   HIPCHK(hipMemcpyAsync(out, d, sizeof(unsigned long long) * nb * 8, hipMemcpyDeviceToHost, e->stream));
+  HIPCHK(hipStreamSynchronize(e->stream));
+  e->allocs.pop_back();
+  (void)hipFree(d);
+  return AZ_OK;
+}
+template <int NT0, int NT1> static int tower_timeline_paired(az_engine* e, int32_t n, unsigned long long* out, int64_t cap) {
+  using T = T16P<ConnectFour, 64, NT0, NT1>;
+  const int nb = (n + T::TB - 1) / T::TB;
+  if (cap < (int64_t)nb * 16) return fail(AZ_ERR_CAPACITY, "need %d words", nb * 16);
+  unsigned long long* d = nullptr;
+  AZCHK(dalloc(e, &d, (size_t)nb * 16));
+  HIPCHK(hipMemsetAsync(d, 0, sizeof(unsigned long long) * nb * 16, e->stream));
+  std::vector<GEnv> envs(n, ConnectFour::init());
+  HIPCHK(hipMemcpyAsync(e->d_tmp_env, envs.data(), sizeof(GEnv) * n, hipMemcpyHostToDevice, e->stream));
+  HIPCHK(hipMemcpyAsync(e->d_ntmp, &n, sizeof(int), hipMemcpyHostToDevice, e->stream));
+  Net16Dev nd = e->net16;
+  HIPCHK(hipFuncSetAttribute(reinterpret_cast<const void*>(&k_tower16x2<ConnectFour, 64, false, NT0, NT1, true>), hipFuncAttributeMaxDynamicSharedMemorySize, T::BYTES));
+  for (int rep = 0; rep < 2; ++rep) {
+    nd.dbg = rep ? d : nullptr;
+    hipLaunchKernelGGL((k_tower16x2<ConnectFour, 64, false, NT0, NT1, true>), dim3(nb), dim3(T::THREADS), T::BYTES, e->stream, nd, e->d_tmp_env, e->d_iota, e->d_ntmp, n, (const float*)nullptr, e->d_hfeat,
+                       (int*)nullptr, 0, e->num_cu);
+  }
+  HIPCHK(hipMemcpyAsync(out, d, sizeof(unsigned long long) * nb * 16, hipMemcpyDeviceToHost, e->stream));
   HIPCHK(hipStreamSynchronize(e->stream));
   e->allocs.pop_back();
   (void)hipFree(d);
@@ -124,7 +147,11 @@
   if (e->cfg.oracle != AZ_ORACLE_RESNET) return fail(AZ_ERR_BAD_ARG, "the tower timeline needs an engine with the ResNet oracle");
   if (!e->net_loaded || n < 1 || n > e->nn_cap) return fail(AZ_ERR_BAD_ARG, "bad n / no net");
   if (e->cfg.game == AZ_GAME_CONNECT_FOUR && e->cfg.net_bf16 && nt == 11) return e->cfg.num_filters == 128 ? tower_timeline_bf16<128>(e, n, out, cap) : tower_timeline_bf16<64>(e, n, out, cap);
-  if (e->cfg.game != AZ_GAME_CONNECT_FOUR || e->cfg.net_bf16 || (nt != 11 && nt != 3 && nt != 2)) return fail(AZ_ERR_BAD_ARG, "connect-four; fp32: nt = 11, 3 or 2 (= split tower), bf16: nt = 11");
+  if (e->cfg.game != AZ_GAME_CONNECT_FOUR || e->cfg.net_bf16 || (nt != 11 && nt != 3 && nt != 2 && nt != 21 && nt != 19)) return fail(AZ_ERR_BAD_ARG, "connect-four; fp32: nt = 11, 3, 2 (= split tower), 21 or 19 (= paired tower), bf16: nt = 11");
+  if (nt == 21 || nt == 19) {
+    if (e->cfg.num_filters != 64) return fail(AZ_ERR_BAD_ARG, "paired tower: 64 filters");
+    return nt == 21 ? tower_timeline_paired<11, 10>(e, n, out, cap) : tower_timeline_paired<10, 9>(e, n, out, cap);
+  }
   if (nt == 2) return e->cfg.num_filters == 128 ? tower_timeline_split(e, n, out, cap) : fail(AZ_ERR_BAD_ARG, "split tower: 128 filters");
   if (e->cfg.num_filters == 64) return nt == 11 ? tower_timeline<64, 11>(e, n, out, cap) : tower_timeline<64, 3>(e, n, out, cap);
   return nt == 11 ? tower_timeline<128, 11>(e, n, out, cap) : tower_timeline<128, 3>(e, n, out, cap);
diff --git a/alphazero.jl_amd/csrc/net_impl.h b/alphazero.jl_amd/csrc/net_impl.h
--- a/alphazero.jl_amd/csrc/net_impl.h
+++ b/alphazero.jl_amd/csrc/net_impl.h
@@ -108,6 +108,14 @@
   for (int i = 0; i < G::RPAD; ++i) out[i] = G::tab.pos[i];
   for (int i = 0; i < 9 * G::RPAD; ++i) out[G::RPAD + i] = G::tab.nbr[i];
   *rows = G::RPAD; *products = G::tab.cost;
+  return AZ_OK;
+}
+template <class T> static int sets_out(int32_t* out, int64_t cap, int* nt0, int* nt1, int* products) {
+  using S = Sets16<typename T::Geo, T::NT0, T::NT1>;
+  if (cap < T::NTW) return fail(AZ_ERR_CAPACITY, "need %d words", T::NTW);
+  for (int k = 0; k < T::NT0; ++k) out[k] = S::sets.tile[0][k];
+  for (int k = 0; k < T::NT1; ++k) out[T::NT0 + k] = S::sets.tile[1][k];
+  *nt0 = T::NT0; *nt1 = T::NT1; products[0] = S::sets.products[0]; products[1] = S::sets.products[1];
   return AZ_OK;
 }
 static const char* game_name(const az_engine* e);
@@ -324,5 +332,10 @@
     return which == 0 ? geometry_out<typename T16<Gm, 64, 11>::Geo>(out, cap, rows, products)                                \
          : which == 1 ? geometry_out<typename T16<Gm, 64, NTS<Gm>>::Geo>(out, cap, rows, products)                                 \
          : which == 2 ? geometry_out<typename T16P<Gm, 64>::Geo>(out, cap, rows, products)                                   \
-                      : geometry_out<typename T16B<Gm, 128, 22>::Geo>(out, cap, rows, products);                             \
-  }
+         : which == 3 ? geometry_out<typename T16B<Gm, 128, 22>::Geo>(out, cap, rows, products)                              \
+                      : geometry_out<typename T16P<Gm, 64, 10, 9>::Geo>(out, cap, rows, products);                           \
+  }                                                                                                                          \
+  int net_sets_##sfx(int which, int32_t* out, int64_t cap, int* nt0, int* nt1, int* products) {                              \
+    return which == 2 ? sets_out<T16P<Gm, 64>>(out, cap, nt0, nt1, products)                                                 \
+                      : sets_out<T16P<Gm, 64, 10, 9>>(out, cap, nt0, nt1, products);                                         \
+  }
diff --git a/alphazero.jl_amd/csrc/resnet16.h b/alphazero.jl_amd/csrc/resnet16.h
--- a/alphazero.jl_amd/csrc/resnet16.h
+++ b/alphazero.jl_amd/csrc/resnet16.h
@@ -221,6 +221,55 @@
   static_assert(NTW == 21 || NTW == 19, "no table slot for this tile count");
   static constexpr int FILT = F;
 };
+template <class G, int NT0, int NT1> struct Sets16 {
+  static_assert(NT0 >= NT1, "set 0 is the larger one");
+  static constexpr int NTW = NT0 + NT1, VMAX = 9 * NTW;
+  struct S {
+    int tile[2][NT0];
+    int products[2];
+  };
+  static constexpr int cost(int t) {
+    int c = 0;
+    for (int tap = 0; tap < 9; ++tap) c += (G::tab.tapmask[t] >> tap) & 1;
+    return c;
+  }
+  static constexpr S make() {
+    bool reach[NT0 + 1][VMAX + 1] = {};
+    bool take[NTW][NT0 + 1][VMAX + 1] = {};
+    reach[0][0] = true;
+    int total = 0;
+    for (int i = 0; i < NTW; ++i) {
+      const int ci = cost(i);
+      total += ci;
+      for (int c = NT0 - 1; c >= 0; --c)
+        for (int v = 0; v + ci <= VMAX; ++v)
+          if (reach[c][v] && !reach[c + 1][v + ci]) { reach[c + 1][v + ci] = true; take[i][c + 1][v + ci] = true; }
+    }
+    int best = -1;
+    for (int v = 0; v <= VMAX; ++v) {
+      if (!reach[NT0][v]) continue;
+      const int d = 2 * v > total ? 2 * v - total : total - 2 * v, db = 2 * best > total ? 2 * best - total : total - 2 * best;
+      if (best < 0 || d < db || (d == db && v > best)) best = v;
+    }
+    S s{};
+    s.products[0] = best; s.products[1] = total - best;
+    int c = NT0, v = best, n1 = NT1;
+    for (int i = NTW - 1; i >= 0; --i) {
+      if (take[i][c][v]) { s.tile[0][--c] = i; v -= cost(i); }
+      else s.tile[1][--n1] = i;
+    }
+    return s;
+  }
+  static constexpr S sets = make();
+};
+template <int NT_, int TILE0> struct TileRange {
+  static constexpr int NT = NT_, DBG_THREAD = 0, DBG_WORDS = 8, DBG_AT = 0;
+  static constexpr int at(int k) { return TILE0 + k; }
+};
+template <class T, int S, bool STAMPS = false> struct TileSet {
+  static constexpr int NT = S ? T::NT1 : T::NT0, DBG_THREAD = S == 0 ? 0 : STAMPS ? T::CT * 64 : -1, DBG_WORDS = 16, DBG_AT = 8 * S;
+  static constexpr int at(int k) { return Sets16<typename T::Geo, T::NT0, T::NT1>::sets.tile[S][k]; }
+};
 
 template <int F> __device__ __forceinline__ int posF(int c) {
   const int G = (c >= F / 2 ? 1 : 0) + 2 * (c & 1), w = (c % (F / 2)) >> 1;
@@ -229,7 +278,8 @@
 
 static constexpr int T16_GMAX = 2;
 
-template <class G, int NT, int TILE0, int KH, int NTAP> struct Steps16 {
+template <class G, class TL, int KH, int NTAP> struct Steps16 {
+  static constexpr int NT = TL::NT;
   static constexpr int MAXS = 9 * KH * ((NT + 1) / 2);
   struct L {
     int n;
@@ -246,14 +296,14 @@
     for (int tap = 0; tap < 9; ++tap) {
       if (NTAP == 1 && tap != 4) continue;
       bool any = false;
-      for (int t = 0; t < NT; ++t) any = any || ((G::tab.tapmask[TILE0 + t] >> tap) & 1);
+      for (int t = 0; t < NT; ++t) any = any || ((G::tab.tapmask[TL::at(t)] >> tap) & 1);
       if (any) taps[ntaps++] = tap;
     }
     for (int ti = 0; ti < ntaps; ++ti) {
       const int tap = taps[ti];
       if (l.first_tap < 0) l.first_tap = (int8_t)tap;
       int act[NT] = {}, na = 0;
-      for (int t = 0; t < NT; ++t) if ((G::tab.tapmask[TILE0 + t] >> tap) & 1) act[na++] = t;
+      for (int t = 0; t < NT; ++t) if ((G::tab.tapmask[TL::at(t)] >> tap) & 1) act[na++] = t;
       for (int kh = 0; kh < KH; ++kh)
         for (int i = 0; i < na; i += 2) {
           const int k = l.n++;
@@ -294,18 +344,25 @@
     if constexpr (T1 >= 0) acc[T1] = __builtin_amdgcn_mfma_f32_16x16x4f32(a[1][q].w, b[q].w, acc[T1], 0, 0, 0);
   }
 }
-template <class T, class SL, int K, int TILE0>
+template <class T, class SL, class TL, int K>
 __device__ __forceinline__ void load_idx16p(const uint16_t* __restrict__ nbr, int lrow, int (&idx)[2]) {
   if constexpr (K < SL::list.n) {
     constexpr int tap = SL::list.tap[K], t0 = SL::list.t0[K], t1 = SL::list.t1[K];
-    idx[0] = (int)nbr[tap * T::RPAD + (TILE0 + t0) * 16 + lrow] * T::STRIDE;
-    if constexpr (t1 >= 0) idx[1] = (int)nbr[tap * T::RPAD + (TILE0 + t1) * 16 + lrow] * T::STRIDE;
-  }
-}
-template <class T, class SL, int NT, int TILE0, int K>
+    constexpr int r0 = TL::at(t0) * 16, r1 = TL::at(t1 >= 0 ? t1 : t0) * 16;
+    idx[0] = (int)nbr[tap * T::RPAD + r0 + lrow] * T::STRIDE;
+    if constexpr (t1 >= 0) idx[1] = (int)nbr[tap * T::RPAD + r1 + lrow] * T::STRIDE;
+  }
+}
+struct NoWarm { static constexpr bool ON = false, MORE = false; };
+template <int SQ, bool MORE_> struct Warm16 {
+  static constexpr bool ON = true, MORE = MORE_;
+  float4 (&b)[SQ];
+  const float4* next;
+};
+template <class T, class SL, class TL, int K, class W>
 __device__ __forceinline__ void conv16p_steps(const float* __restrict__ buf, const uint16_t* __restrict__ nbr, const float4* __restrict__ wl,
-                                              f32x4v (&acc)[NT], int lrow, int g, float4 (&b0)[T::FILT / 16], float4 (&b1)[T::FILT / 16],
-                                              float4 (&aA)[T16_GMAX][4], float4 (&aB)[T16_GMAX][4], int (&idx)[2]) {
+                                              f32x4v (&acc)[TL::NT], int lrow, int g, float4 (&b0)[T::FILT / 16], float4 (&b1)[T::FILT / 16],
+                                              float4 (&aA)[T16_GMAX][4], float4 (&aB)[T16_GMAX][4], int (&idx)[2], const W& w) {
   constexpr int F = T::FILT;
   if constexpr (K < SL::list.n) {
     constexpr int kh = SL::list.kh[K], t0 = SL::list.t0[K], t1 = SL::list.t1[K], ord = SL::list.ord[K];
@@ -317,32 +374,45 @@
       constexpr int ntap = SL::list.next_tap[K];
 #pragma unroll
       for (int q = 0; q < T::SQ; ++q) bn[q] = wl[(size_t)(ntap * T::CT * T::SQ + q) * 64];
+    } else if constexpr (W::MORE && SL::list.first[K]) {
+#pragma unroll
+      for (int q = 0; q < T::SQ; ++q) bn[q] = w.next[(size_t)q * 64];
     }
     if constexpr (K + 1 < SL::list.n) {
       load_rows16p<T>(buf, idx[0], idx[1], SL::list.t1[K + 1] >= 0, SL::list.kh[K + 1], g, nxt);
-      load_idx16p<T, SL, K + 2, TILE0>(nbr, lrow, idx);
-    }
-    mfma_tiles16<t0, t1, kh, F / 16, NT>(cur, bc, acc);
+      load_idx16p<T, SL, TL, K + 2>(nbr, lrow, idx);
+    }
+    mfma_tiles16<t0, t1, kh, F / 16, TL::NT>(cur, bc, acc);
     __builtin_amdgcn_sched_barrier(0);
-    conv16p_steps<T, SL, NT, TILE0, K + 1>(buf, nbr, wl, acc, lrow, g, b0, b1, aA, aB, idx);
-  }
-}
-template <class T, class G, int NT, int TILE0, int NTAP>
+    conv16p_steps<T, SL, TL, K + 1, W>(buf, nbr, wl, acc, lrow, g, b0, b1, aA, aB, idx, w);
+  }
+}
+template <class T, class G, class TL, int NTAP> constexpr int first_tap16() { return NTAP == 1 ? 0 : Steps16<G, TL, T::KH, NTAP>::list.first_tap; }
+template <class T, class G, class TL, int NTAP, class W = NoWarm>
 __device__ __forceinline__ void conv16p(const float* __restrict__ buf, const uint16_t* __restrict__ nbr, const float4* __restrict__ wl,
-                                        f32x4v (&acc)[NT], int lrow, int g) {
+                                        f32x4v (&acc)[TL::NT], int lrow, int g, const W& w = W{}) {
   constexpr int F = T::FILT;
-  using SL = Steps16<G, NT, TILE0, T::KH, NTAP>;
+  using SL = Steps16<G, TL, T::KH, NTAP>;
+  static_assert(!W::ON || SL::list.n > 0, "a warm start hands fragments from convolution to convolution");
   if constexpr (SL::list.n > 0) {
     float4 b0[F / 16], b1[F / 16], aA[T16_GMAX][4], aB[T16_GMAX][4];
     int idx[2] = {0, 0};
-    constexpr int tap0 = NTAP == 1 ? 0 : SL::list.first_tap;
-#pragma unroll
-    for (int q = 0; q < F / 16; ++q) b0[q] = wl[(size_t)(tap0 * T::CT * T::SQ + q) * 64];
-    load_idx16p<T, SL, 0, TILE0>(nbr, lrow, idx);
+    constexpr int tap0 = first_tap16<T, G, TL, NTAP>();
+#pragma unroll
+    for (int q = 0; q < F / 16; ++q) {
+      if constexpr (W::ON) b0[q] = w.b[q];
+      else b0[q] = wl[(size_t)(tap0 * T::CT * T::SQ + q) * 64];
+    }
+    load_idx16p<T, SL, TL, 0>(nbr, lrow, idx);
     load_rows16p<T>(buf, idx[0], idx[1], SL::list.t1[0] >= 0, SL::list.kh[0], g, aA);
-    load_idx16p<T, SL, 1, TILE0>(nbr, lrow, idx);
+    load_idx16p<T, SL, TL, 1>(nbr, lrow, idx);
     __builtin_amdgcn_sched_barrier(0);
-    conv16p_steps<T, SL, NT, TILE0, 0>(buf, nbr, wl, acc, lrow, g, b0, b1, aA, aB, idx);
+    conv16p_steps<T, SL, TL, 0, W>(buf, nbr, wl, acc, lrow, g, b0, b1, aA, aB, idx, w);
+    if constexpr (W::MORE) {
+      constexpr bool in_b0 = SL::list.ord[SL::list.n - 1] & 1;
+#pragma unroll
+      for (int q = 0; q < F / 16; ++q) w.b[q] = in_b0 ? b0[q] : b1[q];
+    }
   }
 }
 
@@ -410,16 +480,23 @@
   }
 };
 
-template <class T, bool FROM_PLANES, int NT, int TILE0, class X = NoXch>
+template <class T, class G, class TL>
+__device__ __forceinline__ const float4* warm_first16(const Net16Dev& net, int l, int cw, int lane) {
+  constexpr size_t LAYER_W = (size_t)9 * T::CT * T::SQ * 64, TAP9 = (size_t)first_tap16<T, G, TL, 9>() * T::CT * T::SQ * 64;
+  return l < 2 * net.nblocks ? net.conv_w + (size_t)l * LAYER_W + (size_t)cw * T::SQ * 64 + lane + TAP9 : net.head_w + (size_t)cw * T::SQ * 64 + lane;
+}
+template <class T, bool FROM_PLANES, class TL, class X = NoXch, bool WARM = false>
 __device__ __forceinline__ void tower16_wave(const Net16Dev& net, float* __restrict__ buf, const float* __restrict__ planes,
                                              const uint16_t* __restrict__ nbr, const uint16_t* __restrict__ pos, int cw,
                                              int lane, int n, int board0, float* __restrict__ hfeat, const X& xch = X{},
                                              int* stop = nullptr, int stop_val = 0) {
   using Gm = typename T::Game;
   using G = typename T::Geo;
-  constexpr int F = T::FILT, P = Gm::P, C = Gm::C, TB = T::TB, STRIDE = T::STRIDE, R0 = TILE0 * 16;
+  constexpr int F = T::FILT, P = Gm::P, C = Gm::C, TB = T::TB, STRIDE = T::STRIDE, NT = TL::NT;
+  struct Rows { int r[NT]; };
+  constexpr Rows R0 = [] { Rows x{}; for (int k = 0; k < NT; ++k) x.r[k] = TL::at(k) * 16; return x; }();
   const int lrow = lane & 15, g = lane >> 4;
-  unsigned long long* dbg = (net.dbg && threadIdx.x == 0) ? net.dbg + (size_t)blockIdx.x * 8 : nullptr;
+  unsigned long long* dbg = (net.dbg && (int)threadIdx.x == TL::DBG_THREAD) ? net.dbg + (size_t)blockIdx.x * TL::DBG_WORDS + TL::DBG_AT : nullptr;
 #define AZ_STAMP16(i) do { if (dbg) dbg[i] = __builtin_readcyclecounter(); } while (0)
   AZ_STAMP16(0);
   const int ch = cw * 16 + lrow;
@@ -444,7 +521,7 @@
       const int tap = kin ? k / C : 4, c = kin ? k % C : 0;
 #pragma unroll
       for (int tile = 0; tile < NT; ++tile) {
-        const int row = kin ? (int)nbr[tap * T::RPAD + R0 + tile * 16 + lrow] : T::RPAD;
+        const int row = kin ? (int)nbr[tap * T::RPAD + R0.r[tile] + lrow] : T::RPAD;
         const float a = planes[row * C + c];
         acc[tile] = __builtin_amdgcn_mfma_f32_16x16x4f32(a, bw, acc[tile], 0, 0, 0);
       }
@@ -456,9 +533,15 @@
       for (int i = 0; i < 4; ++i) {
         const float v = az_fmaf(acc[tile][i], sc, sh);
         const float r = v > 0.0f ? v : 0.0f;
-        buf[(R0 + tile * 16 + g * 4 + i) * STRIDE + oposs] = r;
+        buf[(R0.r[tile] + g * 4 + i) * STRIDE + oposs] = r;
         if (cws == cw) xres[tile][i] = r;
       }
+  }
+  float4 bpre[T::SQ];
+  if constexpr (WARM) {
+    const float4* w0 = warm_first16<T, G, TL>(net, 0, cw, lane);
+#pragma unroll
+    for (int q = 0; q < T::SQ; ++q) bpre[q] = w0[(size_t)q * 64];
   }
   __syncthreads();
   AZ_STAMP16(1);
@@ -469,8 +552,15 @@
     for (int t = 0; t < NT; ++t) acc[t] = f32x4v{0.f, 0.f, 0.f, 0.f};
     int lrow_l = lrow;
     asm volatile("" : "+v"(lrow_l));
-    conv16p<T, G, NT, TILE0, 9>(buf, nbr, net.conv_w + (size_t)layer * LAYER_W + (size_t)cw * T::SQ * 64 + lane, acc, lrow_l, g);
-    const float sc = net.conv_ss[(size_t)layer * 2 * F + ch], sh = net.conv_ss[(size_t)layer * 2 * F + F + ch];
+    float sc, sh;
+    if constexpr (WARM) {
+      sc = net.conv_ss[(size_t)layer * 2 * F + ch]; sh = net.conv_ss[(size_t)layer * 2 * F + F + ch];
+      conv16p<T, G, TL, 9>(buf, nbr, net.conv_w + (size_t)layer * LAYER_W + (size_t)cw * T::SQ * 64 + lane, acc, lrow_l, g,
+                           Warm16<T::SQ, true>{bpre, warm_first16<T, G, TL>(net, layer + 1, cw, lane)});
+    } else {
+      conv16p<T, G, TL, 9>(buf, nbr, net.conv_w + (size_t)layer * LAYER_W + (size_t)cw * T::SQ * 64 + lane, acc, lrow_l, g);
+      sc = net.conv_ss[(size_t)layer * 2 * F + ch]; sh = net.conv_ss[(size_t)layer * 2 * F + F + ch];
+    }
     if (layer == 2) AZ_STAMP16(4);
     if constexpr (X::EARLY_PUBLISH) {
 #pragma unroll
@@ -489,8 +579,8 @@
 #pragma unroll
       for (int tile = 0; tile < NT; ++tile)
 #pragma unroll
-        for (int i = 0; i < 4; ++i) buf[(R0 + tile * 16 + g * 4 + i) * STRIDE + opos] = ov[tile][i];
-      xch.template collect<T, NT, R0>(layer, buf, g, lrow, threadIdx.x);
+        for (int i = 0; i < 4; ++i) buf[(R0.r[tile] + g * 4 + i) * STRIDE + opos] = ov[tile][i];
+      xch.template collect<T, NT, TL::at(0) * 16>(layer, buf, g, lrow, threadIdx.x);
     } else {
     __builtin_amdgcn_s_setprio(2);
     __syncthreads();
@@ -500,7 +590,7 @@
       for (int tile = 0; tile < NT; ++tile)
 #pragma unroll
         for (int i = 0; i < 4; ++i) {
-          const int a = (R0 + tile * 16 + g * 4 + i) * STRIDE + opos;
+          const int a = (R0.r[tile] + g * 4 + i) * STRIDE + opos;
           const float v = az_fmaf(acc[tile][i], sc, sh);
           buf[a] = v > 0.0f ? v : 0.0f;
         }
@@ -509,7 +599,7 @@
       for (int tile = 0; tile < NT; ++tile)
 #pragma unroll
         for (int i = 0; i < 4; ++i) {
-          const int a = (R0 + tile * 16 + g * 4 + i) * STRIDE + opos;
+          const int a = (R0.r[tile] + g * 4 + i) * STRIDE + opos;
           float v = az_fmaf(acc[tile][i], sc, sh);
           v = v + xres[tile][i];
           xres[tile][i] = v > 0.0f ? v : 0.0f;
@@ -525,7 +615,8 @@
   if (stop && threadIdx.x == 0) __hip_atomic_store(stop, stop_val, __ATOMIC_RELAXED, __HIP_MEMORY_SCOPE_AGENT);
 #pragma unroll
   for (int t = 0; t < NT; ++t) acc[t] = f32x4v{0.f, 0.f, 0.f, 0.f};
-  conv16p<T, G, NT, TILE0, 1>(buf, nbr, net.head_w + (size_t)cw * T::SQ * 64 + lane, acc, lrow, g);
+  if constexpr (WARM) conv16p<T, G, TL, 1>(buf, nbr, net.head_w + (size_t)cw * T::SQ * 64 + lane, acc, lrow, g, Warm16<T::SQ, false>{bpre, nullptr});
+  else conv16p<T, G, TL, 1>(buf, nbr, net.head_w + (size_t)cw * T::SQ * 64 + lane, acc, lrow, g);
   {
     const float sc = net.head_ss[ch], sh = net.head_ss[F + ch];
     const int nvalid = ((n - board0) < TB ? (n - board0) : TB) * P;
@@ -533,7 +624,7 @@
     for (int tile = 0; tile < NT; ++tile)
 #pragma unroll
       for (int i = 0; i < 4; ++i) {
-        const int ps = pos[R0 + tile * 16 + g * 4 + i];
+        const int ps = pos[R0.r[tile] + g * 4 + i];
         const float v = az_fmaf(acc[tile][i], sc, sh);
         if (ps < nvalid) hfeat[((size_t)board0 * P + ps) * F + ch] = v > 0.0f ? v : 0.0f;
       }
@@ -581,10 +672,10 @@
   if (board0 >= n) return;
   tower16_fill<T, FROM_PLANES>(buf, planes, nbr, pos, net.geo[T::GEO], leaf_env, eval_slots, X, n, board0, threadIdx.x);
   __syncthreads();
-  tower16_wave<T, FROM_PLANES, NT, 0>(net, buf, planes, nbr, pos, threadIdx.x >> 6, threadIdx.x & 63, n, board0, hfeat);
-}
-
-template <class T, bool FROM_PLANES>
+  tower16_wave<T, FROM_PLANES, TileRange<NT, 0>>(net, buf, planes, nbr, pos, threadIdx.x >> 6, threadIdx.x & 63, n, board0, hfeat);
+}
+
+template <class T, bool FROM_PLANES, bool WARM, bool STAMPS = false>
 __device__ __forceinline__ void tower16x2_body(const Net16Dev& net, const GEnv* __restrict__ leaf_env, const int* __restrict__ eval_slots, int n,
                                                const float* __restrict__ X, float* __restrict__ hfeat, int board0, const uint16_t* __restrict__ geo,
                                                int* stop = nullptr, int stop_val = 0) {
@@ -596,13 +687,13 @@
   tower16_fill<T, FROM_PLANES>(buf, planes, nbr, pos, geo, leaf_env, eval_slots, X, n, board0, threadIdx.x);
   __syncthreads();
   const int wave = threadIdx.x >> 6, lane = threadIdx.x & 63;
-  if (wave < T::CT) tower16_wave<T, FROM_PLANES, T::NT0, 0>(net, buf, planes, nbr, pos, wave, lane, n, board0, hfeat, NoXch{}, stop, stop_val);
-  else tower16_wave<T, FROM_PLANES, T::NT1, T::NT0>(net, buf, planes, nbr, pos, wave - T::CT, lane, n, board0, hfeat);
+  if (wave < T::CT) tower16_wave<T, FROM_PLANES, TileSet<T, 0>, NoXch, WARM>(net, buf, planes, nbr, pos, wave, lane, n, board0, hfeat, NoXch{}, stop, stop_val);
+  else tower16_wave<T, FROM_PLANES, TileSet<T, 1, STAMPS>, NoXch, WARM>(net, buf, planes, nbr, pos, wave - T::CT, lane, n, board0, hfeat);
 }
 __device__ __forceinline__ int* paired_last_round(int* stop, int wg, int nwg, int num_cu) {
   return stop && wg >= (nwg - 1) / num_cu * num_cu ? stop : nullptr;
 }
-template <class Gm, int F, bool FROM_PLANES, int NT0 = 11, int NT1 = 10>
+template <class Gm, int F, bool FROM_PLANES, int NT0 = 11, int NT1 = 10, bool STAMPS = false>
 __global__ void __launch_bounds__(2 * T16Threads<F>::V, 1)
 k_tower16x2(Net16Dev net, const GEnv* __restrict__ leaf_env, const int* __restrict__ eval_slots,
             const int* __restrict__ n_eval_ptr, int n_fixed, const float* __restrict__ X, float* __restrict__ hfeat,
@@ -611,7 +702,7 @@
   const int n = FROM_PLANES ? n_fixed : *n_eval_ptr;
   const int board0 = blockIdx.x * T::TB;
   if (board0 >= n) return;
-  tower16x2_body<T, FROM_PLANES>(net, leaf_env, eval_slots, n, X, hfeat, board0, net.geo[T::GEO], paired_last_round(stop, blockIdx.x, (n + T::TB - 1) / T::TB, num_cu), stop_val);
+  tower16x2_body<T, FROM_PLANES, true, STAMPS>(net, leaf_env, eval_slots, n, X, hfeat, board0, net.geo[T::GEO], paired_last_round(stop, blockIdx.x, (n + T::TB - 1) / T::TB, num_cu), stop_val);
 }
 template <class Gm, int F, bool FROM_PLANES>
 __global__ void __launch_bounds__(2 * T16Threads<F>::V, 1) __attribute__((amdgpu_num_vgpr(88)))
@@ -622,7 +713,7 @@
   const int n = FROM_PLANES ? n_fixed : *n_eval_ptr;
   const int board0 = blockIdx.x * T::TB;
   if (board0 >= n) return;
-  tower16x2_body<T, FROM_PLANES>(net, leaf_env, eval_slots, n, X, hfeat, board0, net.geo[T::GEO], paired_last_round(stop, blockIdx.x, (n + T::TB - 1) / T::TB, num_cu), stop_val);
+  tower16x2_body<T, FROM_PLANES, false>(net, leaf_env, eval_slots, n, X, hfeat, board0, net.geo[T::GEO], paired_last_round(stop, blockIdx.x, (n + T::TB - 1) / T::TB, num_cu), stop_val);
 }
 template <class Gm, int F, bool FROM_PLANES>
 __global__ void __launch_bounds__(2 * T16Threads<F>::V, 1)
@@ -635,12 +726,12 @@
   if ((int)blockIdx.x < first) {
     const int board0 = blockIdx.x * T8::TB;
     if (board0 >= n) return;
-    tower16x2_body<T8, FROM_PLANES>(net, leaf_env, eval_slots, n, X, hfeat, board0, net.geo[T8::GEO],
+    tower16x2_body<T8, FROM_PLANES, true>(net, leaf_env, eval_slots, n, X, hfeat, board0, net.geo[T8::GEO],
                                     n <= first * T8::TB ? stop : nullptr, stop_val);
   } else {
     const int board0 = first * T8::TB + ((int)blockIdx.x - first) * T7::TB;
     if (board0 >= n) return;
-    tower16x2_body<T7, FROM_PLANES>(net, leaf_env, eval_slots, n, X, hfeat, board0, net.geo[T7::GEO], stop, stop_val);
+    tower16x2_body<T7, FROM_PLANES, true>(net, leaf_env, eval_slots, n, X, hfeat, board0, net.geo[T7::GEO], stop, stop_val);
   }
 }
 
@@ -677,7 +768,7 @@
   x.err = err;
   x.hflag = hflag;
   x.pch = ((half ^ 1) * T::CWL + cwl) * 16 + (lane & 15);
-  tower16_wave<T, FROM_PLANES, T::TPW, 0, PairXch>(net, buf, planes, nbr, pos, half * T::CWL + cwl, lane, n, board0, hfeat, x);
+  tower16_wave<T, FROM_PLANES, TileRange<T::TPW, 0>, PairXch>(net, buf, planes, nbr, pos, half * T::CWL + cwl, lane, n, board0, hfeat, x);
 }
 
 struct TrFinal {
@@ -780,7 +871,7 @@
   f32x4v acc[NT];
 #pragma unroll
   for (int t = 0; t < NT; ++t) acc[t] = f32x4v{0.f, 0.f, 0.f, 0.f};
-  conv16p<T, G, NT, 0, 9>(buf, nbr, wfrag + (size_t)wave * T::SQ * 64 + lane, acc, lrow, g);
+  conv16p<T, G, TileRange<NT, 0>, 9>(buf, nbr, wfrag + (size_t)wave * T::SQ * 64 + lane, acc, lrow, g);
   if constexpr (STAMP) { ts[2] = wall_clock64(); __syncthreads(); }
   const int ch = wave * 16 + lrow;
   float* o = out + (size_t)board0 * P * F;
diff --git a/alphazero.jl_amd/csrc/resnet16b.h b/alphazero.jl_amd/csrc/resnet16b.h
--- a/alphazero.jl_amd/csrc/resnet16b.h
+++ b/alphazero.jl_amd/csrc/resnet16b.h
@@ -114,7 +114,7 @@
 template <class T, class G, int NT, int TILE0, int NTAP>
 __device__ __forceinline__ void conv16b(const uint16_t* __restrict__ buf, const uint16_t* __restrict__ nbr, const bf16x8v* __restrict__ wl,
                                         f32x4v (&acc)[NT][2], int lrow, int g) {
-  using SL = Steps16<G, NT, TILE0, 1, NTAP>;
+  using SL = Steps16<G, TileRange<NT, TILE0>, 1, NTAP>;
   if constexpr (SL::list.n > 0) {
     bf16x8v b0[2][T::KS], b1[2][T::KS], aA[2][T::KS], aB[2][T::KS];
     int idx[2] = {0, 0};
```

Measured after the change: 9.011 million (median of 6 runs). No clear change (+0.3%).
